# graz-dev/llms-on-kubernetes

Hardware: AMD Instinct MI355X
Metric: output tok/s through gateway (p50 TTFT reported) (higher is better)
Workload: dtype bf16

## Files before the change

csrc/include/hipserve/kernels.h:

```cpp
#pragma once
#include <hip/hip_runtime.h>
#include <stddef.h>

namespace hipserve {

void launch_embed_rmsnorm(void* out, void* residual, const void* table, const long* ids, const long* src,
                          const long* tok, const void* w, bool weight_f32, int rows, int hidden, float eps,
                          hipStream_t s, float scale = 1.f, void* out8 = nullptr, float* xs8 = nullptr);
void launch_rmsnorm(void* out, void* residual, const void* x, const void* w,
                    bool weight_f32, int rows, int hidden, long x_stride,
                    long out_stride, float eps, hipStream_t s, void* out8 = nullptr, float* xs8 = nullptr);
void launch_qk_rmsnorm(void* qkv, long stride, const float* qw, const float* kw, int T, int nq, int nkv, int D,
                       float eps, hipStream_t s);

void launch_silu_and_mul(void* out, const void* in, long rows, int inter,
                         long in_stride, long out_stride, hipStream_t s);
void launch_gelu_and_mul(void* out, const void* in, long rows, int inter,
                         long in_stride, long out_stride, hipStream_t s);

void launch_rope_cache(void* qkv, long qkv_stride, const long* positions,
                       const long* slots, const float* cos_sin, void* k_cache,
                       void* v_cache, int T, int nq, int nkv, int D,
                       int block_size, int mode, hipStream_t s, bool kv_f8 = false);

size_t paged_decode_smem_bytes(int D);
void launch_paged_decode_qkv(void* out, long out_stride, const float* ws, int S, int N, const long* positions,
                             const long* slots, const float* cos_sin, int mode, void* k_cache, void* v_cache,
                             const int* block_tables, int bt_stride, const int* context_lens, float* tmp_out,
                             float* tmp_ml, int B, int nq, int nkv, int D, int block_size, int part_size,
                             int max_parts, float scale, int window, hipStream_t s, void* out16 = nullptr,
                             const float* qw = nullptr, const float* kw = nullptr, float eps = 1e-6f);
void launch_paged_decode(void* out, long out_stride, const void* q, long q_stride,
                         const void* k_cache, const void* v_cache,
                         const int* block_tables, int bt_stride,
                         const int* context_lens, float* tmp_out, float* tmp_ml,
                         int B, int nq, int nkv, int D, int block_size,
                         int part_size, int max_parts, float scale, int window,
                         hipStream_t s, void* out16 = nullptr, bool kv_f8 = false);

void launch_prefill_attention(void* out, long out_stride, const void* q,
                              long q_stride, const void* k_cache,
                              const void* v_cache, const int* block_tables,
                              int bt_stride, const int* cu_q, const int* ctx_lens,
                              const int* tiles, int ntiles, int nq, int nkv, int D,
                              int block_size, float scale, int window, hipStream_t s, bool kv_f8 = false);

size_t sample_workspace_floats(int rows, int V);
void launch_sample(long* out_tok, float* out_lp, const void* logits, bool is_bf16,
                   long stride, int rows, int V, const float* temperature,
                   const int* top_k, const float* top_p, const long* seeds,
                   const long* steps, float* ws, hipStream_t s, bool two_rounds = true,
                   const float* min_p = nullptr);

void launch_penalty_apply(void* logits, bool is_bf16, long stride, int rows, int V, const int* slot,
                          const float* pres, const float* freq, const float* rep, const int* counts,
                          const unsigned int* seen, hipStream_t s);
void launch_logit_bias_apply(void* logits, bool is_bf16, long stride, int rows, int V, const int* slot,
                             const int* ids, const float* vals, const int* n, int nslots, int width,
                             hipStream_t s);
void launch_penalty_update(const long* tok, const int* slot, int n, int* counts, unsigned int* seen, int V,
                           hipStream_t s);
void launch_penalty_init(int* counts, unsigned int* seen, int V, const int* slots, const int* off,
                         const int* n_prompt, const int* toks, int ninit, hipStream_t s);
void launch_top_logprobs(const void* logits, bool is_bf16, long stride, int rows, int V, const int* nreq,
                         int* out_ids, float* out_lp, int K, hipStream_t s);

void launch_gguf_gemm(void* out, float* ws, const void* x, long x_stride, long out_stride,
                      const void* q, const void* d, const void* m, int qtype, long row_bytes,
                      int M, int N, int K, int splits, hipStream_t s);
void launch_gguf_dequant(void* out, const void* q, const void* d, const void* m, int qtype,
                         long row_bytes, int N, int K, hipStream_t s);
struct GgufPart {
  const void* q;
  const float* rs;
  int qtype;
  int rows;
  int col;
};
void launch_gguf_gemm_parts(void* out, long out_stride, float* ws, const void* x, long x_stride,
                            const GgufPart* parts, int nparts, int M, int Ntot, int K, int S, hipStream_t s,
                            const void* x16 = nullptr);
void launch_gguf_dequant_tiled(void* out, const void* q, const float* rs, int qtype, int N, int K, hipStream_t s,
                               int pack = 0, int nrows = 0, bool kmajor = false);
void launch_fp8_untile(void* out, const void* q, int N, int K, hipStream_t s);
bool launch_gguf_prefill(int epi, void* out, long ldo, const void* x16, const float* rsc, const GgufPart* parts,
                         int nparts, int M, int K, hipStream_t s);
void launch_x_f16_pairs(void* x16, float* rsc, const void* x, long ldx, int M, int K, hipStream_t s);
bool launch_qmoe_gemm(void* out, long out_stride, float* ws, const void* x, long x_stride, const void* q,
                      const float* rs, int qtype, long w_estride, long rs_estride, const int* slots,
                      const int* tile_expert, int tiles_cap, int tile, int gather_k, int N, int K, int S,
                      hipStream_t s, bool kmajor = false, int glu = 0);

}

namespace hipserve {
bool launch_skinny_gemm(void* out, const void* x, long x_stride, const void* w, long out_stride, int M,
                        int N, int K, int rt, int kw, hipStream_t s);

void* car_create(int rank, int world, size_t max_bytes, int nb_large);
void car_get_handle(void* state, void* handle_out);
void car_open(void* state, int peer, const void* handle);
bool car_error(void* state);
void car_destroy(void* state);
size_t car_max_bytes(void* state);
void launch_car(void* state, const void* inp, void* out, size_t bytes, bool two_shot, int blocks, hipStream_t s);
void launch_car_all_gather(void* state, const void* inp, void* out, size_t shard_bytes, size_t row_bytes,
                           hipStream_t s);
bool car_norm_fits(void* state, int M, int N, bool exch_f32);
void launch_car_add_rmsnorm(void* state, void* out, void* residual, const void* x, bool x_f32, int S,
                            const void* w, bool weight_f32, int M, int N, float eps, bool exch_f32, hipStream_t s);

void launch_fill_uniform(void* out, long ld, int rows, int cols, long row0, long col0, long gcols,
                         unsigned int key, float scale, hipStream_t s);

constexpr int DG_GLU = 1, DG_PARTIAL = 2;
bool launch_decode_gemm(void* out, long out_stride, float* ws, const void* x, long x_stride, const void* w, int M,
                        int N, int K, int rt, int S, bool packed, int flags, hipStream_t s);


constexpr int PG_EPI_STORE = 0, PG_EPI_ADD = 1, PG_EPI_GLU = 2, PG_EPI_GEGLU = 3;
constexpr int PW_EPI_STORE = 0, PW_EPI_ADD = 1, PW_EPI_GLU = 2, PW_EPI_GEGLU = 3;
struct PwGroup {
  const int* tile_expert;
  const int* num_tiles;
  long estride;
  const int* gather_slots = nullptr;
  int gather_k = 1;
  int x_rows = 0;
};
bool launch_prefill_gemm_packed(int epi, void* C, long ldc, const void* X, long ldx, const void* Wp, int M, int N,
                                int K, const void* bias, int wm, int grid_req, hipStream_t s,
                                const PwGroup* group = nullptr, int rw = 4);
constexpr int kPgF8Parts = 4;
struct PgF8Part {
  const unsigned char* q;
  const float* rs;
  int rows;
  int tile0;
};
struct PgF8 {
  PgF8Part p[kPgF8Parts];
  int n;
  const float* xs;
};
bool launch_prefill_gemm_f8(int epi, void* C, long ldc, const void* A, long lda, const PgF8& W, int M, int N, int K,
                            hipStream_t s);
bool launch_fp8_decode_gemm(float* ws, const void* xq, const PgF8& W, int M, int N, int K, int S, hipStream_t s);
bool launch_glu_quant(bool gelu, void* out, void* q8, float* xs, const void* in, long rows, int inter,
                      long in_stride, hipStream_t s);
void launch_act_quant_fp8(void* q, float* xs, const void* x, long x_stride, int M, int K, hipStream_t s);

void launch_splitk_add_rmsnorm(void* out, void* residual, const float* ws, int S, const void* w, bool weight_f32,
                               int M, int N, float eps, hipStream_t s, void* out16 = nullptr, void* out8 = nullptr,
                               float* xs8 = nullptr);
void launch_splitk_post_add_rmsnorm(void* out, void* residual, const float* ws, int S, const void* w_post,
                                    const void* w_next, bool weight_f32, int M, int N, float eps, hipStream_t s,
                                    void* out16 = nullptr, void* out8 = nullptr, float* xs8 = nullptr);
void launch_splitk_reduce(void* out, long out_stride, const float* ws, int M, int N, int S, hipStream_t s);
void launch_splitk_glu(void* act, long act_stride, const float* ws, int S, int M, int I, bool gelu, hipStream_t s,
                       void* act16 = nullptr);
void launch_splitk_rope_cache(void* qkv, long qkv_stride, const float* ws, int S, const long* positions,
                              const long* slots, const float* cos_sin, void* k_cache, void* v_cache, int T, int nq,
                              int nkv, int D, int block_size, int mode, hipStream_t s, const void* bias = nullptr,
                              const float* qw = nullptr, const float* kw = nullptr, float eps = 1e-6f,
                              bool kv_f8 = false);
void launch_pack_decode_weight(void* out, const void* w, int N, int K, bool glu, hipStream_t s, int batch = 1);
}

namespace hipserve {
void launch_moe_topk_softmax(const void* logits, bool logits_f32, float* w, int* ids, int T, int E, int k,
                             bool renorm, hipStream_t s, int splits = 0);
void launch_moe_align(const int* ids, int npairs, int E, int tile, int* slots, int slots_cap, int* tile_expert,
                      int tiles_cap, int* num_tiles, int* pair_slot, int* group_end, hipStream_t s,
                      int* hist = nullptr, int expert_lo = 0);
int moe_align_blocks(int npairs);
void launch_moe_gather(void* out, const void* x, long x_stride, const int* slots, int nslots, int k, int H,
// ... 37 lines not shown
```

csrc/kernels/rope_cache.hip:

```cpp
#include <cstdlib>

#include "hipserve/common.h"
#include "hipserve/kernels.h"

namespace hipserve {

template <int kMode>
HS_DEVICE void rotate8(float (&x)[8], float (&y)[8], const float* cs, int i0,
                       int half) {
#pragma unroll
  for (int j = 0; j < 8; ++j) {
    const float c = cs[i0 + j], s = cs[half + i0 + j];
    const float a = x[j], b = y[j];
    rope_rot(a, b, c, s, x[j], y[j]);
  }
}

template <int kMode, typename KV>
__global__ __launch_bounds__(256) void rope_cache_kernel(
    unsigned short* __restrict__ qkv, long qkv_stride,
    const long* __restrict__ positions, const long* __restrict__ slots,
    const float* __restrict__ cos_sin, KV* __restrict__ k_cache,
    KV* __restrict__ v_cache, int nq, int nkv, int D,
    int block_size) {
  const int t = blockIdx.x;
  const long pos = positions[t];
  const long slot = slots[t];
  const int half = D / 2;
  const float* cs = cos_sin + pos * D;
  unsigned short* row = qkv + t * qkv_stride;
  const long blk = slot >= 0 ? slot / block_size : 0;
  const int off = slot >= 0 ? (int)(slot % block_size) : 0;

  if constexpr (kMode == 0) {
    const int chunks = half / 8;
    const int items = (nq + nkv) * chunks;
    for (int it = threadIdx.x; it < items; it += blockDim.x) {
      const int h = it / chunks, c = it % chunks;
      unsigned short* base = row + h * D;
      u16x8 va = *reinterpret_cast<u16x8*>(base + c * 8);
      u16x8 vb = *reinterpret_cast<u16x8*>(base + half + c * 8);
      float x[8], y[8];
#pragma unroll
      for (int j = 0; j < 8; ++j) { x[j] = bf16_to_f32(va[j]); y[j] = bf16_to_f32(vb[j]); }
      rotate8<0>(x, y, cs, c * 8, half);
#pragma unroll
      for (int j = 0; j < 8; ++j) { va[j] = f32_to_bf16(x[j]); vb[j] = f32_to_bf16(y[j]); }
      if (h < nq) {
        *reinterpret_cast<u16x8*>(base + c * 8) = va;
        *reinterpret_cast<u16x8*>(base + half + c * 8) = vb;
      } else if (slot >= 0) {
        const int kh = h - nq;
        KV* kc = k_cache + ((blk * nkv + kh) * block_size + off) * (long)D;
        kv_store8(kc + c * 8, va);
        kv_store8(kc + half + c * 8, vb);
      }
    }
  } else {
    const int chunks = D / 8;
    const int items = (nq + nkv) * chunks;
    for (int it = threadIdx.x; it < items; it += blockDim.x) {
      const int h = it / chunks, c = it % chunks;
      unsigned short* base = row + h * D;
      u16x8 v = *reinterpret_cast<u16x8*>(base + c * 8);
#pragma unroll
      for (int p = 0; p < 4; ++p) {
        const int i = c * 4 + p;
        const float co = cs[i], si = cs[half + i];
        const float a = bf16_to_f32(v[2 * p]), b = bf16_to_f32(v[2 * p + 1]);
        float ra, rb;
        rope_rot(a, b, co, si, ra, rb);
        v[2 * p] = f32_to_bf16(ra);
        v[2 * p + 1] = f32_to_bf16(rb);
      }
      if (h < nq) {
        *reinterpret_cast<u16x8*>(base + c * 8) = v;
      } else if (slot >= 0) {
        const int kh = h - nq;
        KV* kc = k_cache + ((blk * nkv + kh) * block_size + off) * (long)D;
        kv_store8(kc + c * 8, v);
      }
    }
  }
  if (slot >= 0) {
    const unsigned short* vrow = row + (nq + nkv) * D;
    const int chunks = D / 8;
    for (int it = threadIdx.x; it < nkv * chunks; it += blockDim.x) {
      const int kh = it / chunks, c = it % chunks;
      const u16x8 v = *reinterpret_cast<const u16x8*>(vrow + kh * D + c * 8);
      KV* vc = v_cache + (blk * nkv + kh) * (long)D * block_size + off;
#pragma unroll
      for (int j = 0; j < 8; ++j) kv_store1(vc + (c * 8 + j) * block_size, v[j]);
    }
  }
}

constexpr int kRopeTile = 16;

template <int kMode, typename KV>
__global__ __launch_bounds__(256) void rope_cache_tile_kernel(
    unsigned short* __restrict__ qkv, long qkv_stride, const long* __restrict__ positions,
    const long* __restrict__ slots, const float* __restrict__ cos_sin, KV* __restrict__ k_cache,
    KV* __restrict__ v_cache, int T, int nq, int nkv, int D, int block_size, int vfast) {
  extern __shared__ __attribute__((aligned(16))) unsigned short vs[];
  const int t0 = blockIdx.x * kRopeTile;
  const int nt = min(kRopeTile, T - t0);
  const int half = D / 2;
  const int chunks = kMode == 0 ? half / 8 : D / 8;
  const int nh = nq + nkv;
  const int per_tok = chunks * 2;
  for (int it = threadIdx.x; it < nt * per_tok; it += blockDim.x) {
    const int tt = it / per_tok, c = (it % per_tok) >> 1, hpar = it & 1;
    const int t = t0 + tt;
    const long pos = positions[t];
    const long slot = slots[t];
    const float* cs = cos_sin + pos * D;
    unsigned short* row = qkv + t * qkv_stride;
    const long blk = slot >= 0 ? slot / block_size : 0;
    const int off = slot >= 0 ? (int)(slot % block_size) : 0;
    if constexpr (kMode == 0) {
      float co[8], si[8];
#pragma unroll
      for (int j = 0; j < 8; ++j) { co[j] = cs[c * 8 + j]; si[j] = cs[half + c * 8 + j]; }
      for (int h0 = hpar; h0 < nh; h0 += 8) {
        u16x8 va[4], vb[4];
#pragma unroll
        for (int q = 0; q < 4; ++q) {
          const int h = min(h0 + 2 * q, nh - 1);
          va[q] = *reinterpret_cast<const u16x8*>(row + h * D + c * 8);
          vb[q] = *reinterpret_cast<const u16x8*>(row + h * D + half + c * 8);
        }
#pragma unroll
        for (int q = 0; q < 4; ++q) {
          const int h = h0 + 2 * q;
          if (h >= nh || (h >= nq && slot < 0)) continue;
#pragma unroll
          for (int j = 0; j < 8; ++j) {
            float ra, rb;
            rope_rot(bf16_to_f32(va[q][j]), bf16_to_f32(vb[q][j]), co[j], si[j], ra, rb);
            va[q][j] = f32_to_bf16(ra);
            vb[q][j] = f32_to_bf16(rb);
          }
          if (h < nq) {
            *reinterpret_cast<u16x8*>(row + h * D + c * 8) = va[q];
            *reinterpret_cast<u16x8*>(row + h * D + half + c * 8) = vb[q];
          } else {
            KV* dst = k_cache + ((blk * nkv + (h - nq)) * block_size + off) * (long)D;
            kv_store8(dst + c * 8, va[q]);
            kv_store8(dst + half + c * 8, vb[q]);
          }
        }
      }
    } else {
      float co[4], si[4];
#pragma unroll
      for (int p = 0; p < 4; ++p) { co[p] = cs[c * 4 + p]; si[p] = cs[half + c * 4 + p]; }
      for (int h0 = hpar; h0 < nh; h0 += 8) {
        u16x8 v[4];
#pragma unroll
        for (int q = 0; q < 4; ++q)
          v[q] = *reinterpret_cast<const u16x8*>(row + min(h0 + 2 * q, nh - 1) * D + c * 8);
#pragma unroll
        for (int q = 0; q < 4; ++q) {
          const int h = h0 + 2 * q;
          if (h >= nh || (h >= nq && slot < 0)) continue;
#pragma unroll
          for (int p = 0; p < 4; ++p) {
            float ra, rb;
            rope_rot(bf16_to_f32(v[q][2 * p]), bf16_to_f32(v[q][2 * p + 1]), co[p], si[p], ra, rb);
            v[q][2 * p] = f32_to_bf16(ra);
            v[q][2 * p + 1] = f32_to_bf16(rb);
          }
          if (h < nq) *reinterpret_cast<u16x8*>(row + h * D + c * 8) = v[q];
          else kv_store8(k_cache + ((blk * nkv + (h - nq)) * block_size + off) * (long)D + c * 8, v[q]);
        }
      }
    }
  }
  const int VW = nkv * D, VR = VW + 8;
  const int vchunks = VW / 8;
  for (int it = threadIdx.x; it < nt * vchunks; it += blockDim.x) {
    const int tt = it / vchunks, c = it % vchunks;
    *reinterpret_cast<u16x8*>(vs + tt * VR + c * 8) =
        *reinterpret_cast<const u16x8*>(qkv + (t0 + tt) * qkv_stride + (nq + nkv) * D + c * 8);
  }
  __syncthreads();
  const long s0 = slots[t0];
  const int off0 = s0 >= 0 ? (int)(s0 % block_size) : 1;
  bool contig = vfast && nt == kRopeTile && (block_size & 7) == 0 && (off0 & 7) == 0 && off0 + kRopeTile <= block_size;
  for (int i = 1; contig && i < kRopeTile; ++i) contig = slots[t0 + i] == s0 + i;
  if (contig) {
    const long blk = s0 / block_size;
    for (int it = threadIdx.x; it < 2 * VW; it += blockDim.x) {
      const int r = it >> 1, hl = it & 1;
      const int kh = r / D, d = r % D;
      u16x8 v;
#pragma unroll
      for (int j = 0; j < 8; ++j) v[j] = vs[(hl * 8 + j) * VR + r];
      kv_store8(v_cache + (blk * nkv + kh) * (long)D * block_size + (long)d * block_size + off0 + hl * 8, v);
    }
    return;
  }
  const int tt = threadIdx.x & (kRopeTile - 1);
  const long slot = tt < nt ? slots[t0 + tt] : -1;
  if (slot < 0) return;
  const long blk = slot / block_size;
  const int off = (int)(slot % block_size);
  for (int r = threadIdx.x / kRopeTile; r < VW; r += blockDim.x / kRopeTile) {
    const int kh = r / D, d = r % D;
    kv_store1(v_cache + (blk * nkv + kh) * (long)D * block_size + (long)d * block_size + off, vs[tt * VR + r]);
  }
}

static bool rope_tile_enabled() {
  static const bool on = [] {
    const char* e = getenv("HIPSERVE_ROPE_TILE");
    return !(e && atoi(e) == 0);
  }();
  return on;
}

static int rope_vfast() {
  static const int on = [] {
    const char* e = getenv("HIPSERVE_ROPE_VFAST");
    return !(e && atoi(e) == 0) ? 1 : 0;
  }();
  return on;
}

template <typename KV>
static void rope_cache_t(unsigned short* q, long qkv_stride, const long* positions, const long* slots,
                         const float* cos_sin, KV* kc, KV* vc, int T, int nq, int nkv, int D, int block_size,
                         int mode, hipStream_t s) {
  if (T >= 2048 && nkv * D <= 2048 && rope_tile_enabled()) {
    const dim3 tg((T + kRopeTile - 1) / kRopeTile);
    const size_t smem = (size_t)kRopeTile * (nkv * D + 8) * sizeof(unsigned short);
    if (mode == 0)
      rope_cache_tile_kernel<0, KV><<<tg, 256, smem, s>>>(q, qkv_stride, positions, slots, cos_sin, kc, vc, T, nq,
                                                          nkv, D, block_size, rope_vfast());
    else
      rope_cache_tile_kernel<1, KV><<<tg, 256, smem, s>>>(q, qkv_stride, positions, slots, cos_sin, kc, vc, T, nq,
                                                          nkv, D, block_size, rope_vfast());
    return;
  }
  if (mode == 0)
    rope_cache_kernel<0, KV><<<T, 256, 0, s>>>(q, qkv_stride, positions, slots, cos_sin, kc, vc, nq, nkv, D,
                                               block_size);
  else
    rope_cache_kernel<1, KV><<<T, 256, 0, s>>>(q, qkv_stride, positions, slots, cos_sin, kc, vc, nq, nkv, D,
                                               block_size);
}

void launch_rope_cache(void* qkv, long qkv_stride, const long* positions,
                       const long* slots, const float* cos_sin, void* k_cache,
                       void* v_cache, int T, int nq, int nkv, int D,
                       int block_size, int mode, hipStream_t s, bool kv_f8) {
  if (T <= 0) return;
  auto* q = static_cast<unsigned short*>(qkv);
  if (kv_f8)
    rope_cache_t(q, qkv_stride, positions, slots, cos_sin, static_cast<unsigned char*>(k_cache),
                 static_cast<unsigned char*>(v_cache), T, nq, nkv, D, block_size, mode, s);
  else
    rope_cache_t(q, qkv_stride, positions, slots, cos_sin, static_cast<unsigned short*>(k_cache),
                 static_cast<unsigned short*>(v_cache), T, nq, nkv, D, block_size, mode, s);
}

}
```

csrc/torch_bindings.cpp:

```cpp
#include <torch/library.h>
#include <ATen/ATen.h>
#include <ATen/hip/impl/HIPGuardImplMasqueradingAsCUDA.h>
#include <ATen/hip/impl/HIPStreamMasqueradingAsCUDA.h>

#include <initializer_list>
#include <sstream>
#include <type_traits>

#include "hipserve/kernels.h"
#include "hipserve/quant_formats.h"

namespace {

hipStream_t cur_stream() {
  return c10::hip::getCurrentHIPStreamMasqueradingAsCUDA().stream();
}


enum : unsigned { BF16 = 1, F32 = 2, F16 = 4, U8 = 8, I8 = 16, I16 = 32, I32 = 64, I64 = 128, F8 = 256, OTHER = 512 };
constexpr unsigned BYTES = U8 | I8 | F8, ANYTYPE = ~0u;
struct DtypeName { unsigned bit; at::ScalarType type; const char* name; };
const DtypeName kDtypes[] = {{BF16, at::kBFloat16, "bf16"}, {F32, at::kFloat, "fp32"},  {F16, at::kHalf, "f16"},
                             {U8, at::kByte, "uint8"},      {I8, at::kChar, "int8"},    {I16, at::kShort, "int16"},
                             {I32, at::kInt, "int32"},      {I64, at::kLong, "int64"},  {F8, at::kFloat8_e4m3fn, "float8_e4m3fn"}};
// ... 221 lines not shown
    const int n = rs[i].numel();
    W.p[i] = hipserve::PgF8Part{a.as<uint8_t>(q[i], "q[i] (tiled FP8 [N/16, K/256, 4096] with rs [N])", CONTIG,
                                              exactly((int64_t)n * K)),
                                a.as<float>(rs[i], "rs[i]", CONTIG), n, tile0 ? rows / 256 : 0};
    rows += n;
  }
  return rows;
}

using hipserve::gq::QuantFormat;

std::string quant_formats() {
  std::ostringstream o;
  for (int id : hipserve::gq::kQuantFormatIds) {
    const QuantFormat f = hipserve::gq::quant_format(id);
    o << f.name << ' ' << f.id << ' ' << f.chunk_bytes << ' ' << f.sub_shift << ' ' << f.gguf << ' ' << f.row_scaled
      << ' ' << f.prefill << ' ' << f.moe << '\n';
  }
  return o.str();
}
QuantFormat tiled_format(int64_t qtype, const char* op, bool moe = false) {
  const QuantFormat f = hipserve::gq::quant_format(qtype == (int)qtype ? (int)qtype : -1);
  TORCH_CHECK(f.id >= 0 && (f.moe || !moe), op, ": kernel qtype ", qtype, moe ? " has no expert body" : " is unknown",
              "; name id chunk sub_shift gguf row_scaled prefill moe:\n", quant_formats());
  return f;
}

long tiled_parts(const Args& a, const std::vector<at::Tensor>& qs, const std::vector<at::Tensor>* rss,
                 const std::vector<int64_t>& qtypes, const std::vector<int64_t>& rows, const std::vector<int64_t>& cols,
                 int64_t K, hipserve::GgufPart* P) {
  const size_t np = qs.size();
  TORCH_CHECK(np >= 1 && np <= 4 && qtypes.size() == np && (!rss || rss->size() == np) && rows.size() == np &&
              cols.size() == np, a.op, ": 1-4 parts");
  long span = 0;
  for (size_t i = 0; i < np; ++i) {
    const QuantFormat f = tiled_format(qtypes[i], a.op);
    TORCH_CHECK(cols[i] >= 0 && cols[i] % 4 == 0 && rows[i] % 16 == 0 && rows[i] > 0, a.op,
                ": parts are 16-row multiples at 4-aligned columns");
    const void* q = a.ptr(qs[i], "qs[i] (a tiled [N/16, K/256, chunk] tensor of its format)", U8, CONTIG,
                          exactly(rows[i] / 16 * (K / 256) * f.chunk_bytes));
    const float* rs = rss && f.row_scaled ? a.as<float>((*rss)[i], "rss[i] (FP8 / INT8C: an fp32 scale per row)",
                                                         CONTIG, exactly(rows[i]))
                                          : nullptr;
    P[i] = hipserve::GgufPart{q, rs, (int)qtypes[i], (int)rows[i], (int)cols[i]};
    span = std::max(span, (long)(cols[i] + rows[i]));
  }
  return span;
}

struct GemmOut { void* out = nullptr; long stride = 0; float* ws = nullptr; };
GemmOut partials_or_out(const Args& a, const at::Tensor& out, const at::Tensor& ws, int64_t S, int64_t rows, int64_t N,
                        int64_t out_cols) {
  GemmOut o;
  o.ws = a.as_if<float>(ws, "ws", CONTIG, ws.numel() > 0 ? S * rows * N : 0);
  if (o.ws) return o;
  TORCH_CHECK(S == 1, a.op, ": split-K needs a partial workspace");
  o.out = a.ptr(out, "out", BF16, ROWS4, {rows, at_least(out_cols)});
  o.stride = out.stride(0);
  return o;
}

struct DecodeX { const void* p; int M, K; long stride; };
DecodeX decode_gemm_x(const Args& a, const at::Tensor& x, int64_t splits) {
  const void* p = a.ptr(x, "x", BF16, ROWS8, {ANY, ANY});
  const int M = x.size(0), K = x.size(1);
  TORCH_CHECK(M >= 1 && M <= 64, a.op, ": 1 <= M <= 64");
  TORCH_CHECK(splits >= 1 && K % (256 * splits) == 0, a.op, ": K must be a multiple of 256*splits");
  return {p, M, K, (long)x.stride(0)};
}

struct MoeTiles { int *slots, *tile_expert; long nslots; int tiles_cap; };
MoeTiles moe_tiles(const Args& a, const at::Tensor& slots, const at::Tensor& tile_expert, int64_t tile) {
  TORCH_CHECK(tile > 0, a.op, ": tile > 0");
  int* sp = a.as<int>(slots, "slots", CONTIG);
  const long nslots = slots.numel();
  return {sp, a.as<int>(tile_expert, "tile_expert", CONTIG, (nslots + tile - 1) / tile), nslots, (int)tile_expert.numel()};
}

struct Combine { const float* w; const int* pair_slot; };
Combine combine_args(const Args& a, const at::Tensor& w, const at::Tensor& pair_slot, int64_t pairs) {
  return {a.as<float>(w, "w", CONTIG, pairs), a.as<int>(pair_slot, "pair_slot", CONTIG, pairs)};
}

struct PenState { int* counts; unsigned int* seen; int V; };
PenState pen_state(const Args& a, const at::Tensor& counts, const at::Tensor& seen) {
  int* c = a.as<int>(counts, "counts", CONTIG, {ANY, ANY});
  const int V = counts.size(1);
  return {c, reinterpret_cast<unsigned int*>(a.as<int>(seen, "seen", CONTIG, {counts.size(0), (V + 31) / 32})), V};
}


void rmsnorm_op(const char* name, at::Tensor& out, const at::Tensor& x, at::Tensor* residual, const at::Tensor& weight,
                double eps, const c10::optional<at::Tensor>& out8, const c10::optional<at::Tensor>& xs8) {
  Args a(name, x, "x");
  const void* xp = a.ptr(x, "x", BF16, ROWS, {ANY, ANY});
  const int rows = x.size(0), hidden = x.size(1);
  TORCH_CHECK(hidden % 8 == 0 && hidden <= 16384, name, ": hidden must be a multiple of 8, <= 16384");
  void* op = a.ptr(out, "out", BF16, ROWS, {at_least(rows), at_least(hidden)});
  void* rp = residual ? a.ptr(*residual, "residual", BF16, CONTIG, {rows, hidden}) : nullptr;
  const NormWeight w = norm_weight(a, weight, "weight", hidden);
  const E4m3Out o8 = e4m3_out_args(a, out8, xs8, out);
  hipserve::launch_rmsnorm(op, rp, xp, w.p, w.f32, rows, hidden, x.stride(0), out.stride(0), (float)eps,
                           cur_stream(), o8.q, o8.xs);
}
void rmsnorm(at::Tensor& out, const at::Tensor& x, const at::Tensor& weight, double eps,
             const c10::optional<at::Tensor>& out8, const c10::optional<at::Tensor>& xs8) {
  rmsnorm_op("rmsnorm", out, x, nullptr, weight, eps, out8, xs8);
}
void fused_add_rmsnorm(at::Tensor& out, const at::Tensor& x, at::Tensor& residual, const at::Tensor& weight, double eps,
                       const c10::optional<at::Tensor>& out8, const c10::optional<at::Tensor>& xs8) {
  rmsnorm_op("fused_add_rmsnorm", out, x, &residual, weight, eps, out8, xs8);
}

void embed_rmsnorm(at::Tensor& out, at::Tensor& residual, const at::Tensor& table, const at::Tensor& ids,
                   const c10::optional<at::Tensor>& src, const c10::optional<at::Tensor>& tok,
                   const at::Tensor& weight, double eps, double scale, const c10::optional<at::Tensor>& out8,
                   const c10::optional<at::Tensor>& xs8) {
  Args a("embed_rmsnorm", table, "table");
  const void* tp = a.ptr(table, "table", BF16, CONTIG, {ANY, ANY});
  const int64_t* idp = a.as<int64_t>(ids, "ids", CONTIG);
  const int hidden = table.size(1), rows = ids.numel();
  TORCH_CHECK(hidden % 8 == 0 && hidden <= 16384, "embed_rmsnorm: hidden must be a multiple of 8, <= 16384");
  void* op = a.ptr(out, "out", BF16, CONTIG, {rows, hidden});
  void* rp = a.ptr(residual, "residual", BF16, CONTIG, {rows, hidden});
  TORCH_CHECK(src.has_value() == tok.has_value(), "embed_rmsnorm: src and tok come together");
  const int64_t *sp = nullptr, *kp = nullptr;
  if (src.has_value()) {
    sp = a.as<int64_t>(*src, "src", CONTIG, exactly(rows));
    kp = a.as<int64_t>(*tok, "tok", CONTIG);
  }
  const NormWeight w = norm_weight(a, weight, "weight", hidden);
  const E4m3Out o8 = e4m3_out_args(a, out8, xs8, out);
  hipserve::launch_embed_rmsnorm(op, rp, tp, idp, sp, kp, w.p, w.f32, rows, hidden, (float)eps, cur_stream(),
                                 (float)scale, o8.q, o8.xs);
}

using GluLauncher = void (*)(void*, const void*, long, int, long, long, hipStream_t);
void glu_and_mul(const char* name, GluLauncher launch, at::Tensor& out, const at::Tensor& x) {
  Args a(name, x, "x");
  const void* xp = a.ptr(x, "x", BF16, ROWS, {ANY, ANY});
  TORCH_CHECK(x.size(1) % 16 == 0, name, ": x [rows, 2 I], I % 8 == 0");
  void* op = a.ptr(out, "out", BF16, ROWS, {x.size(0), x.size(1) / 2});
  launch(op, xp, x.size(0), out.size(1), x.stride(0), out.stride(0), cur_stream());
}
void silu_and_mul(at::Tensor& out, const at::Tensor& x) {
  glu_and_mul("silu_and_mul", &hipserve::launch_silu_and_mul, out, x);
}
void gelu_and_mul(at::Tensor& out, const at::Tensor& x) {
  glu_and_mul("gelu_and_mul", &hipserve::launch_gelu_and_mul, out, x);
}

void rope_cache(at::Tensor& qkv, const at::Tensor& positions, const at::Tensor& slots,
                const at::Tensor& cos_sin, at::Tensor& k_cache, at::Tensor& v_cache,
                int64_t nq, int64_t nkv, int64_t head_dim, int64_t mode) {
  Args a("rope_cache", qkv, "qkv");
  TORCH_CHECK(head_dim > 0 && head_dim % 16 == 0 && (mode == 0 || mode == 1), "rope_cache: head_dim % 16 == 0, mode 0 / 1");
  void* qp = a.ptr(qkv, "qkv", BF16, ROWS, {ANY, at_least((nq + 2 * nkv) * head_dim)});
  const int T = qkv.size(0);
  const RopeArgs r = rope_args(a, positions, slots, cos_sin, T, head_dim);
  const KvCache kv = kv_cache(a, k_cache, v_cache, nkv, head_dim);
  hipserve::launch_rope_cache(qp, qkv.stride(0), r.positions, r.slots, r.cos_sin, kv.k, kv.v, T, nq, nkv, head_dim,
                              kv.bs, mode, cur_stream(), kv.f8);
}

void paged_decode(at::Tensor& out, const at::Tensor& q, const at::Tensor& k_cache,
                  const at::Tensor& v_cache, const at::Tensor& block_tables,
                  const at::Tensor& context_lens, at::Tensor& tmp_out, at::Tensor& tmp_ml,
                  int64_t nq, int64_t nkv, int64_t part_size, double scale, int64_t window,
                  const c10::optional<at::Tensor>& out16) {
  Args a("paged_decode", q, "q");
  const KvCache kv = kv_cache(a, k_cache, v_cache, nkv);
  const int D = kv.D;
  TORCH_CHECK(D == 64 || D == 96 || D == 128 || D == 256, "paged_decode: head_dim 64/96/128/256");
  const void* qp = a.ptr(q, "q", BF16, ROWS, {ANY, at_least(nq * D)});
  const int B = q.size(0);
  void* op = a.ptr(out, "out", BF16, ROWS, {at_least(B), at_least(nq * D)});
  const DecodeAttn g = decode_attn_args(a, block_tables, context_lens, tmp_out, tmp_ml, B, nq, nkv, D, kv.bs,
                                        part_size, window);
  hipserve::launch_paged_decode(op, out.stride(0), qp, q.stride(0), kv.k, kv.v, g.block_tables, g.bt_stride,
                                g.context_lens, g.tmp_out, g.tmp_ml, B, nq, nkv, D, kv.bs, part_size, g.max_parts,
                                (float)scale, (int)window, cur_stream(), out16_arg(a, out16, out), kv.f8);
}

void paged_decode_qkv(at::Tensor& out, const at::Tensor& ws, int64_t splits, const at::Tensor& positions,
                      const at::Tensor& slots, const at::Tensor& cos_sin, at::Tensor& k_cache, at::Tensor& v_cache,
                      const at::Tensor& block_tables, const at::Tensor& context_lens, at::Tensor& tmp_out,
                      at::Tensor& tmp_ml, int64_t nq, int64_t nkv, int64_t part_size, double scale, int64_t window,
                      int64_t mode, const c10::optional<at::Tensor>& out16, const c10::optional<at::Tensor>& q_w,
                      const c10::optional<at::Tensor>& k_w, double eps) {
  Args a("paged_decode_qkv", ws, "ws");
  const KvCache kv = kv_cache(a, k_cache, v_cache, nkv);
  const int D = kv.D;
  TORCH_CHECK(!kv.f8, "paged_decode_qkv: bf16 KV cache only");
  TORCH_CHECK(D == 64 || D == 128, "paged_decode_qkv: head_dim 64/128");
  TORCH_CHECK(mode == 0 || mode == 1, "paged_decode_qkv: mode 0 / 1");
  const float *qwp, *kwp;
  if (qk_norm_weights(a, q_w, k_w, D, &qwp, &kwp))
    TORCH_CHECK(mode == 0, "paged_decode_qkv: q/k norm needs rotate-half RoPE (mode 0)");
  void* op = a.ptr(out, "out", BF16, ROWS, {ANY, at_least(nq * D)});
  const int B = out.size(0);
  const long N = (nq + 2 * nkv) * D;
  const float* wsp = splitk_ws(a, ws, splits, B, N);
  const RopeArgs r = rope_args(a, positions, slots, cos_sin, B, D);
  const DecodeAttn g = decode_attn_args(a, block_tables, context_lens, tmp_out, tmp_ml, B, nq, nkv, D, kv.bs,
                                        part_size, window);
  hipserve::launch_paged_decode_qkv(op, out.stride(0), wsp, splits, N, r.positions, r.slots, r.cos_sin, mode, kv.k,
                                    kv.v, g.block_tables, g.bt_stride, g.context_lens, g.tmp_out, g.tmp_ml, B, nq,
                                    nkv, D, kv.bs, part_size, g.max_parts, (float)scale, (int)window, cur_stream(),
                                    out16_arg(a, out16, out), qwp, kwp, (float)eps);
}

void prefill_attention(at::Tensor& out, const at::Tensor& q, const at::Tensor& k_cache,
                       const at::Tensor& v_cache, const at::Tensor& block_tables,
                       const at::Tensor& cu_q, const at::Tensor& ctx_lens,
                       const at::Tensor& tiles, int64_t nq, int64_t nkv, double scale, int64_t window) {
  Args a("prefill_attention", q, "q");
  const KvCache kv = kv_cache(a, k_cache, v_cache, nkv);
  const int D = kv.D;
  TORCH_CHECK(D == 64 || D == 96 || D == 128 || D == 256, "prefill_attention: head_dim 64/96/128/256");
  TORCH_CHECK(window >= 0, "prefill_attention: window >= 0");
  TORCH_CHECK(kv.bs % 16 == 0 && nq % nkv == 0, "prefill_attention: block_size % 16 == 0, nq % nkv == 0");
  const void* qp = a.ptr(q, "q", BF16, ROWS, {ANY, at_least(nq * D)});
  void* op = a.ptr(out, "out", BF16, ROWS, {ANY, at_least(nq * D)});
  const int* bt = a.as<int>(block_tables, "block_tables", ROWS, {ANY, ANY});
  const int* cu = a.as<int>(cu_q, "cu_q", ROWS);
  const int* cl = a.as<int>(ctx_lens, "ctx_lens", ROWS);
  const int* tp = a.as<int>(tiles, "tiles", CONTIG, {ANY, 2});
  hipserve::launch_prefill_attention(op, out.stride(0), qp, q.stride(0), kv.k, kv.v, bt, block_tables.stride(0), cu, cl,
                                     tp, tiles.size(0), nq, nkv, D, kv.bs, (float)scale, (int)window, cur_stream(),
                                     kv.f8);
}

void qk_rmsnorm(at::Tensor& qkv, const at::Tensor& q_w, const at::Tensor& k_w, int64_t nq, int64_t nkv,
                int64_t head_dim, double eps) {
  Args a("qk_rmsnorm", qkv, "qkv");
  TORCH_CHECK(head_dim > 0 && head_dim <= 256, "qk_rmsnorm: head_dim <= 256");
  void* qp = a.ptr(qkv, "qkv", BF16, ROWS, {ANY, at_least((nq + nkv) * head_dim)});
  const float* qw = a.as<float>(q_w, "q_w", CONTIG, exactly(head_dim));
  const float* kw = a.as<float>(k_w, "k_w", CONTIG, exactly(head_dim));
  hipserve::launch_qk_rmsnorm(qp, qkv.stride(0), qw, kw, qkv.size(0), nq, nkv, head_dim, (float)eps, cur_stream());
}

void sample(at::Tensor& out_tok, at::Tensor& out_lp, const at::Tensor& logits,
            const at::Tensor& temperature, const at::Tensor& top_k, const at::Tensor& top_p,
            const at::Tensor& seeds, const at::Tensor& steps, bool two_rounds,
            const c10::optional<at::Tensor>& min_p) {
  Args a("sample", logits, "logits");
  const Logits L = logits_rows(a, logits);
  const int rows = L.rows;
  int64_t* tok = a.as<int64_t>(out_tok, "out_tok", CONTIG, rows);
  float* lp = a.as_if<float>(out_lp, "out_lp", CONTIG, out_lp.numel() > 0 ? rows : 0);
  const float* temp = a.as<float>(temperature, "temperature", CONTIG, rows);
  const int* tk = a.as<int>(top_k, "top_k", CONTIG, rows);
  const float* tpp = a.as<float>(top_p, "top_p", CONTIG, rows);
  const int64_t* sd = a.as<int64_t>(seeds, "seeds", CONTIG, rows);
  const int64_t* st = a.as<int64_t>(steps, "steps", CONTIG, rows);
  const float* minp = maybe(min_p).defined() ? a.as<float>(*min_p, "min_p", CONTIG, rows) : nullptr;
  const size_t wsn = hipserve::sample_workspace_floats(rows, L.V);
  at::Tensor ws;
  if (wsn) ws = at::empty({(long)wsn}, logits.options().dtype(at::kFloat));
  hipserve::launch_sample(tok, lp, L.p, L.bf16, L.stride, rows, L.V, temp, tk, tpp, sd, st,
                          wsn ? a.as<float>(ws, "workspace", CONTIG) : nullptr, cur_stream(), two_rounds, minp);
}

void gguf_gemm(at::Tensor& out, const at::Tensor& x, const at::Tensor& q, const at::Tensor& d,
               const at::Tensor& mn, int64_t qtype, int64_t row_bytes, int64_t N, int64_t K,
               at::Tensor& ws, int64_t splits) {
  Args a("gguf_gemm", x, "x");
  TORCH_CHECK(K > 0 && K % 256 == 0, "gguf_gemm: K must be a multiple of 256");
  TORCH_CHECK(qtype >= 0 && qtype <= 6, "gguf_gemm: qtype 0..6");
  const void* xp = a.ptr(x, "x", BF16, ROWS8, {ANY, at_least(K)});
  const int M = x.size(0);
  TORCH_CHECK(M <= 64, "gguf_gemm handles M <= 64 (use gguf_dequant + GEMM above)");
  void* op = a.ptr(out, "out", BF16, ROWS, {M, at_least(N)});
  const void* qp = a.ptr(q, "q", U8, CONTIG);
  const void* dp = a.ptr_if(d, "d (SoA scales)", I16 | F16, CONTIG, qtype <= 2 ? N * (K / 32) : 0);
  const void* mp = a.ptr_if(mn, "m (SoA mins)", I16 | F16, CONTIG, qtype == 1 ? N * (K / 32) : 0);
  float* wp = splits > 1 ? splitk_ws(a, ws, splits, M, N) : nullptr;
  hipserve::launch_gguf_gemm(op, wp, xp, x.stride(0), out.stride(0), qp, dp, mp, qtype, row_bytes, M, N, K, splits,
                             cur_stream());
}

int64_t gguf_gemm_parts(at::Tensor& out, at::Tensor& ws, const at::Tensor& x, const std::vector<at::Tensor>& qs,
                        const std::vector<at::Tensor>& rss, const std::vector<int64_t>& qtypes, const std::vector<int64_t>& rows,
                        const std::vector<int64_t>& cols, int64_t Ntot, int64_t K, int64_t splits,
                        const c10::optional<at::Tensor>& x16) {
  Args a("gguf_gemm_parts", x, "x");
  TORCH_CHECK(K > 0 && K % 256 == 0 && splits >= 1, "gguf_gemm_parts: K % 256 == 0, splits >= 1");
  const void* xp = a.ptr(x, "x", BF16, ROWS8, {ANY, at_least(K)});
  const int M = x.size(0);
  TORCH_CHECK(M >= 1, "gguf_gemm_parts: M >= 1 (M > 64 sweeps 64-row tiles)");
  const int nsb = K / 256;
  const int per = (nsb + splits - 1) / splits;
  const int S = (nsb + per - 1) / per;
  hipserve::GgufPart P[4];
  TORCH_CHECK(tiled_parts(a, qs, &rss, qtypes, rows, cols, K, P) <= Ntot, "gguf_gemm_parts: parts must lie inside Ntot");
  const GemmOut o = partials_or_out(a, out, ws, S, M, Ntot, Ntot);
  const void* x16p = f16_twin(a, x16, "x16", x, at_least(K));
  hipserve::launch_gguf_gemm_parts(o.out, o.stride, o.ws, xp, x.stride(0), P, (int)qs.size(), M, Ntot, K, splits,
                                   cur_stream(), x16p);
  return S;
}

void x_f16_pairs(at::Tensor& x16, at::Tensor& rsc, const at::Tensor& x) {
  Args a("x_f16_pairs", x, "x");
  const void* xp = a.ptr(x, "x", BF16, ROWS8, {ANY, ANY});
  const int M = x.size(0);
  void* x16p = a.ptr(x16, "x16", F16, CONTIG, {M, ANY});
  const int K = x16.size(1);
  TORCH_CHECK(K % 8 == 0 && x.size(1) >= K, "x_f16_pairs: x16 [M, K], K % 8, x rows of >= K");
  float* rp = a.as<float>(rsc, "rsc", CONTIG, M);
  if (M == 0) return;
  hipserve::launch_x_f16_pairs(x16p, rp, xp, x.stride(0), M, K, cur_stream());
}

// ... 516 lines not shown
  at::Tensor hist;
  if (nb > 1) hist = at::empty({(long)nb * 128}, ids.options().dtype(at::kInt));
  hipserve::launch_moe_align(ip, npairs, E, tile, t.slots, t.nslots, t.tile_expert,
                             t.tiles_cap, ntp, psp, ge, cur_stream(), nb > 1 ? a.as<int>(hist, "histogram", CONTIG) : nullptr,
                             (int)expert_lo);
}

void moe_gather(at::Tensor& out, const at::Tensor& x, const at::Tensor& slots, int64_t k) {
  Args a("moe_gather", x, "x");
  const int* sp = a.as<int>(slots, "slots", CONTIG);
  void* op = a.ptr(out, "out", BF16, CONTIG, {at_least(slots.numel()), ANY});
  const int H = out.size(1);
  const void* xp = a.ptr(x, "x", BF16, ROWS8, {ANY, H});
  TORCH_CHECK(H % 8 == 0, "moe_gather: H % 8 == 0");
  hipserve::launch_moe_gather(op, xp, x.stride(0), sp, slots.numel(), k, H, cur_stream());
}

void moe_gemm(at::Tensor& out, const at::Tensor& x, const at::Tensor& w, const at::Tensor& slots,
              const at::Tensor& tile_expert, int64_t tile, int64_t gather_k) {
  Args a("moe_gemm", x, "x");
  const void* wp = a.ptr(w, "w", BF16, CONTIG, {ANY, ANY, ANY});
  const int N = w.size(1), K = w.size(2);
  TORCH_CHECK(K % 256 == 0, "moe_gemm: K % 256 == 0");
  const MoeTiles t = moe_tiles(a, slots, tile_expert, tile);
  const void* xp = a.ptr(x, "x", BF16, ROWS8, {ANY, at_least(K)});
  void* op = a.ptr(out, "out", BF16, ROWS, {at_least(t.nslots), at_least(N)});
  TORCH_CHECK(gather_k > 0 || x.size(0) >= t.nslots, "moe_gemm: ungathered x needs one row per slot");
  hipserve::launch_moe_gemm(op, out.stride(0), xp, x.stride(0), wp, t.slots, t.tile_expert, t.nslots / tile, tile,
                            gather_k, N, K, cur_stream());
}

void moe_combine(at::Tensor& out, const at::Tensor& y, const at::Tensor& w, const at::Tensor& pair_slot,
                 int64_t k) {
  Args a("moe_combine", y, "y");
  void* op = a.ptr(out, "out", BF16, CONTIG, {ANY, ANY});
  const int T = out.size(0), H = out.size(1);
  TORCH_CHECK(H % 8 == 0, "moe_combine: H % 8 == 0");
  const void* yp = a.ptr(y, "y", BF16, CONTIG, {ANY, H});
  const Combine c = combine_args(a, w, pair_slot, T * k);
  hipserve::launch_moe_combine(op, yp, c.w, c.pair_slot, T, k, H, cur_stream());
}

void moe_decode_gemm(at::Tensor& out, const at::Tensor& x, const at::Tensor& w, const at::Tensor& slots,
                     const at::Tensor& tile_expert, int64_t tile, int64_t gather_k, int64_t N, int64_t splits,
                     bool packed, bool glu) {
  Args a("moe_decode_gemm", x, "x");
  TORCH_CHECK(tile == 16 || tile == 32 || tile == 64, "moe_decode_gemm: tile in {16, 32, 64}");
  const void* xp = a.ptr(x, "x", BF16, ROWS8, {ANY, ANY});
  const long K = x.size(1);
  TORCH_CHECK(K % 256 == 0 && splits >= 1 && K % (256 * splits) == 0, "moe_decode_gemm: K must be a multiple of 256 * splits");
  const MoeTiles t = moe_tiles(a, slots, tile_expert, tile);
  TORCH_CHECK(t.nslots % tile == 0, "moe_decode_gemm: slots in whole tiles");
  const void* wp = a.ptr(w, "w", BF16, CONTIG);
  TORCH_CHECK(w.dim() >= 2, "moe_decode_gemm: w [E, ...]");
  const long estride = packed ? (N + 127) / 128 * 128 * K : N * K;
  TORCH_CHECK(w.numel() == w.size(0) * estride, "moe_decode_gemm: weight size != E * (packed) N * K");
  TORCH_CHECK(gather_k > 0 || x.size(0) >= t.nslots, "moe_decode_gemm: ungathered x needs one row per slot");
  void* op;
  float* ws = nullptr;
  long out_stride = N;
  if (a.check(out, "out", F32 | BF16, ROWS) == F32) {
    TORCH_CHECK(!glu && N % 4 == 0, "moe_decode_gemm: fp32 partials [splits, slots, N] take no glu, N % 4 == 0");
    op = ws = a.as<float>(out, "out (fp32 partials [splits, slots, N])", CONTIG, splits * t.nslots * N);
    if (out.dim() == 2) out_stride = out.stride(0);
  } else {
    TORCH_CHECK(splits == 1, "moe_decode_gemm: bf16 out [slots, N] (glu: [slots, N/2]) needs splits == 1");
    TORCH_CHECK(!glu || N % 128 == 0, "moe_decode_gemm: glu needs N % 128 == 0");
    op = a.ptr(out, "out", BF16, ROWS4, {at_least(t.nslots), at_least(glu ? N / 2 : N)});
    out_stride = out.stride(0);
  }
  TORCH_CHECK(hipserve::launch_moe_decode_gemm(op, out_stride, ws, xp, x.stride(0), wp, estride, t.slots, t.tile_expert,
                                               t.nslots / tile, tile, gather_k, N, K, splits, packed, glu, cur_stream()),
              "moe_decode_gemm: unsupported K / splits (K / splits / 256 in {1,2,3,4,6,7,8,16}) or glu without packing");
}

void moe_combine_partial(at::Tensor& out, const at::Tensor& ws, const at::Tensor& w, const at::Tensor& pair_slot,
                         int64_t k) {
  Args a("moe_combine_partial", ws, "ws");
  void* op = a.ptr(out, "out", BF16, CONTIG, {ANY, ANY});
  const int T = out.size(0), H = out.size(1);
  TORCH_CHECK(H % 8 == 0, "moe_combine_partial: H % 8 == 0");
  const float* wsp = a.as<float>(ws, "ws", CONTIG, {ANY, ANY, H});
  const Combine c = combine_args(a, w, pair_slot, T * k);
  hipserve::launch_moe_combine_partial(op, wsp, ws.stride(0), ws.size(0), c.w, c.pair_slot, T, k, H, cur_stream());
}

void moe_combine_add_rmsnorm(at::Tensor& out, at::Tensor& residual, const at::Tensor& y, int64_t splits,
                             const at::Tensor& w, const at::Tensor& pair_slot, int64_t k, const at::Tensor& norm_w,
                             double eps) {
  Args a("moe_combine_add_rmsnorm", y, "y");
  void* op = a.ptr(out, "out", BF16, CONTIG, {ANY, ANY});
  const int T = out.size(0), H = out.size(1);
  TORCH_CHECK(H % 8 == 0 && H <= 16384, "moe_combine_add_rmsnorm: H must be a multiple of 8, <= 16384");
  void* rp = a.ptr(residual, "residual", BF16, CONTIG, {T, H});
  const Combine c = combine_args(a, w, pair_slot, T * k);
  const NormWeight nw = norm_weight(a, norm_w, "norm_w", H);
  const void* yp = splits > 0 ? a.ptr(y, "y (fp32 partials [S, slots, H])", F32, CONTIG, {at_least(splits), ANY, H})
                              : a.ptr(y, "y", BF16, CONTIG, {ANY, H});
  const long slab = splits > 0 ? y.stride(0) : 0;
  hipserve::launch_moe_combine_add_rmsnorm(op, rp, yp, slab, (int)splits, c.w, c.pair_slot, T, k, H, nw.p, nw.f32,
                                           (float)eps, cur_stream());
}

void layernorm(at::Tensor& out, const at::Tensor& x, const at::Tensor& w, const at::Tensor& b,
               const c10::optional<at::Tensor>& residual, double eps) {
  Args a("layernorm", x, "x");
  const void* xp = a.ptr(x, "x", BF16, CONTIG, {ANY, ANY});
  const int rows = x.size(0), C = x.size(1);
  TORCH_CHECK(C % 8 == 0 && C <= 8192, "layernorm: C must be a multiple of 8, <= 8192");
  void* op = a.ptr(out, "out", BF16, CONTIG, {rows, C});
  const void* wp = a.ptr(w, "w", BF16, CONTIG, exactly(C));
  const void* bp = a.ptr(b, "b", BF16, CONTIG, exactly(C));
  void* rp = maybe(residual).defined() ? a.ptr(*residual, "residual", BF16, CONTIG, {rows, C}) : nullptr;
  hipserve::launch_layernorm(op, rp, xp, wp, bp, rows, C, (float)eps, cur_stream());
}

void gelu_(at::Tensor& x, bool tanh_approx) {
  Args a("gelu_", x, "x");
  void* xp = a.ptr(x, "x", BF16, CONTIG);
  TORCH_CHECK(x.numel() % 8 == 0, "gelu_: numel must be a multiple of 8");
  hipserve::launch_gelu(xp, x.numel(), tanh_approx, cur_stream());
}

void vision_attention(at::Tensor& out, at::Tensor& qkv, const at::Tensor& cos_sin, const at::Tensor& cu,
                      const at::Tensor& tiles, int64_t nh, int64_t D, double scale) {
  Args a("vision_attention", qkv, "qkv");
  TORCH_CHECK(D == 16 || D == 64 || D == 72 || D == 80 || D == 96 || D == 128,
              "vision_attention: head_dim must be one of 16, 64, 72, 80, 96, 128");
  void* qp = a.ptr(qkv, "qkv", BF16, CONTIG, {ANY, 3 * nh * D});
  const int T = qkv.size(0);
  void* op = a.ptr(out, "out", BF16, CONTIG, {T, nh * D});
  const float* cs = a.as<float>(cos_sin, "cos_sin", CONTIG, {at_least(T), D});
  const int* cup = a.as<int>(cu, "cu", CONTIG);
  const int* tp = a.as<int>(tiles, "tiles", CONTIG, {ANY, 2});
  hipserve::launch_vision_attention(op, qp, cs, cup, tp, tiles.size(0), T, nh, D, (float)scale, cur_stream());
}

}

#define GPU_KEY_OPS(X) \
  X(moe_topk_softmax, "(Tensor(a!) w, Tensor(b!) ids, Tensor logits, int k, bool renorm=True, int splits=0) -> ()") \
  X(moe_combine_add_rmsnorm, "(Tensor(a!) out, Tensor(b!) residual, Tensor y, int splits, Tensor w, Tensor pair_slot, int k, Tensor norm_w, float eps) -> ()") \
  X(moe_align, "(Tensor ids, int E, int tile, Tensor(a!) slots, Tensor(b!) tile_expert, Tensor(c!) num_tiles, Tensor(d!) pair_slot, Tensor(e!)? group_end=None, int expert_lo=0) -> ()") \
  X(moe_gather, "(Tensor(a!) out, Tensor x, Tensor slots, int k) -> ()") \
  X(moe_gemm, "(Tensor(a!) out, Tensor x, Tensor w, Tensor slots, Tensor tile_expert, int tile, int gather_k) -> ()") \
  X(moe_combine, "(Tensor(a!) out, Tensor y, Tensor w, Tensor pair_slot, int k) -> ()") \
  X(moe_decode_gemm, "(Tensor(a!) out, Tensor x, Tensor w, Tensor slots, Tensor tile_expert, int tile, int gather_k, int N, int splits, bool packed, bool glu) -> ()") \
  X(moe_combine_partial, "(Tensor(a!) out, Tensor ws, Tensor w, Tensor pair_slot, int k) -> ()") \
  X(rmsnorm, "(Tensor(a!) out, Tensor x, Tensor weight, float eps, Tensor(b!)? out8=None, Tensor(c!)? xs8=None) -> ()") \
  X(embed_rmsnorm, "(Tensor(a!) out, Tensor(b!) residual, Tensor table, Tensor ids, Tensor? src, Tensor? tok, " \
                   "Tensor weight, float eps, float scale=1.0, Tensor(c!)? out8=None, Tensor(d!)? xs8=None) -> ()") \
  X(fused_add_rmsnorm, "(Tensor(a!) out, Tensor x, Tensor(b!) residual, Tensor weight, float eps, Tensor(c!)? out8=None, Tensor(d!)? xs8=None) -> ()") \
  X(silu_and_mul, "(Tensor(a!) out, Tensor x) -> ()") \
  X(rope_cache, "(Tensor(a!) qkv, Tensor positions, Tensor slots, Tensor cos_sin, Tensor(b!) k_cache, Tensor(c!) v_cache, int nq, int nkv, int head_dim, int mode) -> ()") \
  X(paged_decode, "(Tensor(a!) out, Tensor q, Tensor k_cache, Tensor v_cache, Tensor block_tables, Tensor context_lens, Tensor(b!) tmp_out, Tensor(c!) tmp_ml, int nq, int nkv, int part_size, float scale, int window=0, Tensor(d!)? out16=None) -> ()") \
  X(prefill_attention, "(Tensor(a!) out, Tensor q, Tensor k_cache, Tensor v_cache, Tensor block_tables, Tensor cu_q, Tensor ctx_lens, Tensor tiles, int nq, int nkv, float scale, int window=0) -> ()") \
  X(qk_rmsnorm, "(Tensor(a!) qkv, Tensor q_w, Tensor k_w, int nq, int nkv, int head_dim, float eps) -> ()") \
  X(gelu_and_mul, "(Tensor(a!) out, Tensor x) -> ()") \
  X(gguf_gemm, "(Tensor(a!) out, Tensor x, Tensor q, Tensor d, Tensor m, int qtype, int row_bytes, int N, int K, Tensor(b!) ws, int splits) -> ()") \
  X(gguf_dequant, "(Tensor(a!) out, Tensor q, Tensor d, Tensor m, int qtype, int row_bytes, int N, int K) -> ()") \
  X(fill_uniform, "(Tensor(a!) out, int row0, int col0, int gcols, int key, float scale) -> ()") \
  X(decode_gemm, "(Tensor(a!) out, Tensor x, Tensor w, Tensor(b!) ws, int rt, int splits) -> ()") \
  X(decode_gemm_packed, "(Tensor(a!) out, Tensor x, Tensor wp, Tensor(b!) ws, int N, int rt, int splits) -> ()") \
  X(pack_decode_weight, "(Tensor(a!) out, Tensor w, bool glu=False) -> ()") \
  X(decode_gemm_partial, "(Tensor(a!) ws, Tensor x, Tensor w, int N, int rt, int splits, bool packed) -> ()") \
  X(decode_gemm_glu, "(Tensor(a!) act, Tensor x, Tensor wp, Tensor(b!) ws, int N, int rt, int splits) -> ()") \
  X(prefill_gemm_packed, "(Tensor(a!) out, Tensor x, Tensor wp, int N, int epi, Tensor? bias=None, int wm=1, int grid=0, int rw=4) -> ()") \
  X(prefill_gemm_packed_grouped, "(Tensor(a!) out, Tensor x, Tensor wp, int N, int epi, Tensor tile_expert, Tensor num_tiles, int wm=1, int rw=4, Tensor? gather_slots=None, int gather_k=1) -> ()") \
  X(prefill_gemm_f8, "(Tensor(a!) out, Tensor xq, Tensor xs, Tensor[] q, Tensor[] rs, int epi) -> ()") \
  X(fp8_decode_gemm, "(Tensor(a!) ws, Tensor xq, Tensor xs, Tensor[] q, Tensor[] rs, int splits) -> ()") \
  X(glu_quant, "(Tensor(a!)? out, Tensor(b!) q8, Tensor(c!) xs, Tensor x, bool gelu) -> ()") \
  X(act_quant_fp8, "(Tensor(a!) xq, Tensor(b!) xs, Tensor x) -> ()") \
  X(splitk_add_rmsnorm, "(Tensor(a!) out, Tensor(b!) residual, Tensor ws, int splits, Tensor weight, float eps, Tensor(c!)? out16=None, Tensor(d!)? out8=None, Tensor(e!)? xs8=None) -> ()") \
  X(splitk_post_add_rmsnorm, "(Tensor(a!) out, Tensor(b!) residual, Tensor ws, int splits, Tensor w_post, Tensor w_next, float eps, Tensor(c!)? out16=None, Tensor(d!)? out8=None, Tensor(e!)? xs8=None) -> ()") \
  X(splitk_glu, "(Tensor(a!) act, Tensor ws, int splits, bool gelu, Tensor(b!)? act16=None) -> ()") \
  X(paged_decode_qkv, "(Tensor(a!) out, Tensor ws, int splits, Tensor positions, Tensor slots, Tensor cos_sin, Tensor(b!) k_cache, Tensor(c!) v_cache, Tensor block_tables, Tensor context_lens, Tensor(d!) tmp_out, Tensor(e!) tmp_ml, int nq, int nkv, int part_size, float scale, int window, int mode, Tensor(f!)? out16=None, Tensor? q_norm=None, Tensor? k_norm=None, float eps=1e-6) -> ()") \
  X(splitk_reduce, "(Tensor(a!) out, Tensor ws, int splits) -> ()") \
  X(splitk_rope_cache, "(Tensor(a!) qkv, Tensor ws, int splits, Tensor positions, Tensor slots, Tensor cos_sin, Tensor(b!) k_cache, Tensor(c!) v_cache, int nq, int nkv, int head_dim, int mode, Tensor? bias=None, Tensor? q_w=None, Tensor? k_w=None, float eps=1e-6) -> ()") \
  X(skinny_gemm, "(Tensor(a!) out, Tensor x, Tensor w, int rt, int kw) -> ()") \
  X(penalty_apply, "(Tensor(a!) logits, Tensor slot, Tensor pres, Tensor freq, Tensor rep, Tensor counts, Tensor seen) -> ()") \
  X(logit_bias_apply, "(Tensor(a!) logits, Tensor slot, Tensor ids, Tensor vals, Tensor n) -> ()") \
  X(penalty_update, "(Tensor tok, Tensor slot, Tensor(a!) counts, Tensor(b!) seen) -> ()") \
  X(penalty_init, "(Tensor(a!) counts, Tensor(b!) seen, Tensor slots, Tensor off, Tensor n_prompt, Tensor toks) -> ()") \
  X(top_logprobs, "(Tensor logits, Tensor nreq, Tensor(a!) out_ids, Tensor(b!) out_lp) -> ()") \
  X(layernorm, "(Tensor(a!) out, Tensor x, Tensor w, Tensor b, Tensor(b!)? residual, float eps) -> ()") \
  X(gelu_, "(Tensor(a!) x, bool tanh_approx) -> ()") \
  X(vision_attention, "(Tensor(a!) out, Tensor(b!) qkv, Tensor cos_sin, Tensor cu, Tensor tiles, int nh, int D, float scale) -> ()") \
  X(sample, "(Tensor(a!) out_tok, Tensor(b!) out_lp, Tensor logits, Tensor temperature, Tensor top_k, Tensor top_p, Tensor seeds, Tensor steps, bool two_rounds=True, Tensor? min_p=None) -> ()")

TORCH_LIBRARY(hipserve, m) {
#define DEF_OP(name, schema) m.def(#name schema);
  GPU_KEY_OPS(DEF_OP)
#undef DEF_OP
  m.def("gguf_gemm_parts(Tensor(a!) out, Tensor(b!) ws, Tensor x, Tensor[] qs, Tensor[] rss, int[] qtypes, int[] rows, int[] cols, int Ntot, int K, int splits, Tensor? x16=None) -> int", &gguf_gemm_parts);
  m.def("gguf_prefill(Tensor(a!) out, Tensor x16, Tensor rsc, Tensor[] qs, int[] qtypes, int[] rows, int[] cols, int K, int epi) -> bool", &gguf_prefill);
  m.def("x_f16_pairs(Tensor(a!) x16, Tensor(b!) rsc, Tensor x) -> ()", &x_f16_pairs);
  m.def("gguf_dequant_tiled(Tensor(a!) out, Tensor q, Tensor rs, int qtype, int N, int K, int pack=0, int nrows=0, bool kmajor=False) -> ()",
        &gguf_dequant_tiled);
  m.def("fp8_untile(Tensor(a!) out, Tensor q, int N, int K) -> ()", &fp8_untile);
  m.def("quant_formats() -> str", &quant_formats);
  m.def("qmoe_gemm(Tensor(a!) out, Tensor(b!) ws, Tensor x, Tensor q, Tensor rs, int qtype, int N, int K, Tensor slots, Tensor tile_expert, int tile, int gather_k, int splits, bool kmajor=False, int glu=0) -> int", &qmoe_gemm);
  m.def("stage_copy(Tensor(a!)[] dst, Tensor[] src, int device) -> ()", &stage_copy);
  m.def("car_create(int rank, int world, int max_bytes, int nb_large=512) -> int", &car_create);
  m.def("car_handle(int state) -> Tensor", &car_handle);
  m.def("car_open(int state, int peer, Tensor handle) -> ()", &car_open);
  m.def("car_all_reduce(int state, Tensor inp, Tensor(a!) out, bool two_shot) -> ()", &car_all_reduce);
  m.def("car_all_gather(int state, Tensor inp, Tensor(a!) out) -> ()", &car_all_gather);
  m.def("car_norm_fits(int state, int M, int N, bool exch_f32) -> bool", &car_norm_fits);
  m.def("car_add_rmsnorm(int state, Tensor(a!) out, Tensor(b!) residual, Tensor x, int splits, Tensor weight, float eps, bool exch_f32) -> ()", &car_add_rmsnorm);
  m.def("car_error(int state) -> bool", &car_error);
  m.def("car_destroy(int state) -> ()", &car_destroy);
}

TORCH_LIBRARY_IMPL(hipserve, CUDA, m) {
#define IMPL_OP(name, schema) m.impl(#name, &name);
  GPU_KEY_OPS(IMPL_OP)
#undef IMPL_OP
}
```

hipserve/engine/model_runner.py:

```python
from __future__ import annotations

import logging
import math
import os
import time
from dataclasses import dataclass, field

import numpy as np
import torch

from ..config import EngineConfig, ModelConfig
from ..models.llama import AttnMeta, LlamaModel
from ..ops import get_ops
from ..parallel.comm import TPGroup
from ..runtime import native
from .request import MAX_LOGIT_BIAS
from .scheduler import SchedulerOutput

log = logging.getLogger("hipserve.runner")
PREFILL_TILE = 128
TOP_LOGPROBS = 20
GPU_HEAD_DIMS = (64, 96, 128, 256)
GRAPH_BUCKETS = [1, 2, 4, 8, 16, 24, 32, 48, 64, 80, 96, 112, 128, 160, 192, 224, 256, 320, 384, 448, 512]


@dataclass
class StepInputs:
    ids: np.ndarray
    positions: np.ndarray
    slots: np.ndarray
    num_prefill_tokens: int
    num_decode: int
    bt_prefill: np.ndarray | None
    cu_q: np.ndarray | None
    ctx_prefill: np.ndarray | None
    tiles: np.ndarray | None
    bt_decode: np.ndarray | None
    ctx_decode: np.ndarray | None
    logits_rows: np.ndarray
    temperature: np.ndarray
    top_k: np.ndarray
    top_p: np.ndarray
    seeds: np.ndarray
    steps: np.ndarray
    pen_slot: np.ndarray | None = None
    pen_vals: np.ndarray | None = None
    nlogprobs: np.ndarray | None = None
    pen_init: tuple | None = None
    top_logprobs: int = 0
    src: np.ndarray | None = None
    extra: dict = field(default_factory=dict)
    min_p: np.ndarray | None = None
    bias_slot: np.ndarray | None = None
    bias_init: tuple | None = None


def pad_table(times: dict, tol: float = 1.03) -> dict:
    pad, best_t, best_m = {}, float("inf"), None
    for m in sorted(times, reverse=True):
        if times[m] <= best_t * tol:
            best_t, best_m = min(times[m], best_t), m
        pad[m] = best_m
    return {m: p for m, p in pad.items() if p > m}


_PACKED_TIMING: dict = {}


class ModelRunner:
    def __init__(self, ecfg: EngineConfig, mcfg: ModelConfig, tp: TPGroup, device=None):
        self.ecfg = ecfg
        self.mcfg = mcfg
        self.tp = tp
        self.device = torch.device(device or tp.device or ecfg.device)
        if self.device.type == "cuda":
            if self.device.index is None:
                self.device = torch.device("cuda", torch.cuda.current_device())
            torch.cuda.set_device(self.device)
        self.dtype = {"bfloat16": torch.bfloat16, "bf16": torch.bfloat16, "auto": torch.bfloat16,
                      "float32": torch.float32, "fp32": torch.float32}[ecfg.dtype]
        if self.device.type == "cuda" and self.dtype != torch.bfloat16:
            raise ValueError("the gfx950 kernels run bf16 activations; use --dtype bfloat16")
        if self.device.type == "cuda" and mcfg.head_dim not in GPU_HEAD_DIMS:
            raise ValueError(f"{mcfg.name}: head_dim {mcfg.head_dim} has no gfx950 attention kernel "
                             f"(supported: {', '.join(map(str, GPU_HEAD_DIMS))})")
        self.ops = get_ops(self.device)
        self.max_model_len = min(ecfg.max_model_len or mcfg.max_position_embeddings,
                                 mcfg.max_position_embeddings)
        self.block_size = ecfg.block_size
        self.model = LlamaModel(mcfg, tp, self.device, self.dtype, self.ops, max_pos=self.max_model_len,
                                enable_expert_parallel=ecfg.enable_expert_parallel)
        if mcfg.num_experts and tp.world_size > 1:
            m = self.model
            log.info("rank %d/%d MoE sharding: %s (experts %d-%d of %d, width %d of %d)", tp.rank, tp.world_size,
                     m.moe_shard[0], m.expert_lo, m.expert_lo + m.num_local_experts - 1, mcfg.num_experts,
                     m.inter, mcfg.expert_size)
        self.model.decode_partition = ecfg.decode_partition
        self.model.block_size_hint = ecfg.block_size
        if ecfg.kv_fp8:
            self.model.kv_dtype = torch.float8_e4m3fn
            self.model.fused_qkv_attention = False
        t0 = time.time()
        self._load_weights()
        self.load_time = time.time() - t0
        from ..utils.faults import FaultInjector

        FaultInjector.from_env().on_init(tp.rank, tp.world_size)
        self.init_times = {"weights_s": round(self.load_time, 2)}
        t1 = time.time()
        if tp.world_size > 1:
            if "tp_exact_reduce" in ecfg.extra:
                tp.exact_reduce = bool(ecfg.extra["tp_exact_reduce"])
            if self.device.type == "cuda":
                H = mcfg.hidden_size
                msg = max(ecfg.max_num_batched_tokens * H * 2,
                          ecfg.max_num_seqs * self.model.vpad * 2, 8 << 20)
                if tp.ensure_custom_ar(msg):
                    tp.calibrate_collectives(H, ecfg.max_num_batched_tokens)
        self.init_times["collectives_s"] = round(time.time() - t1, 2)
        self.max_bs = min(ecfg.max_num_seqs, max(GRAPH_BUCKETS))
        self.buckets = [b for b in GRAPH_BUCKETS if b <= max(self.max_bs, 1)]
        if self.buckets[-1] < self.max_bs:
            self.buckets.append(self.max_bs)
        tp.rccl_floor_rows = max(tp.rccl_floor_rows, self.buckets[-1])
        t1 = time.time()
        self.gemm_report = []
        if self.device.type == "cuda" and ecfg.extra.get("gemm_autotune", True):
            from ..ops import gemm

            ms = [b for b in self.buckets if b <= 64]
            self.model.fused_decode = bool(ecfg.extra.get("fused_decode",
                                                          os.environ.get("HIPSERVE_FUSED_DECODE", "1") != "0"))
            fused = self.model.fused_gemm_shapes() if self.model.fused_decode else {}
            self.gemm_report = gemm.TUNER.tune(self.model.gemm_shapes(), self.device, ms, fused=fused)
            self.single_layout = None
            if ecfg.extra.get("packed_decode", True):
                why = self._single_layout_reason()
                if why:
                    n, freed = self.model.to_single_layout()
                    self.single_layout = {"reason": why, "weights": n, "row_major_gb_freed": round(freed / 2**30, 2)}
                else:
                    self.model.pack_decode_weights(gemm.TUNER.packed_shapes())
            shadow = ecfg.extra.get("quant_dense_shadow", os.environ.get("HIPSERVE_QUANT_SHADOW", "0") == "1")
            moes = self.model.quant_moes() if hasattr(self.model, "quant_moes") else []
            if moes and shadow:
                from ..ops import quant as Q

                total = torch.cuda.get_device_properties(self.device).total_memory
                self.quant_shadow_bytes = Q.make_moe_shadows(moes, self.device, (24 << 30) + total // 4)
            qws = self.model.quant_weights() if hasattr(self.model, "quant_weights") else []
            if qws:
                from ..ops import quant as Q

                self.gguf_split_report = Q.tune_splits(
                    qws, self.device, [m for m in Q.M_BUCKETS if m <= 64],
                    f8_ms=[m for m in Q.F8_M_BUCKETS if m <= max(64, max(self.buckets, default=1))])
                lm = getattr(self.model, "lm_head", None)
                self.qprefill_report = Q.tune_qprefill([w for w in qws if w is not lm], self.device,
                                                       min(ecfg.max_num_batched_tokens, 8192)) \
                    if Q.QPREFILL_MODE == "auto" else []
                total = torch.cuda.get_device_properties(self.device).total_memory
                self.quant_shadow_bytes = getattr(self, "quant_shadow_bytes", 0)
                if shadow:
                    gguf = ecfg.extra.get("gguf_dense_shadow", shadow)
                    self.quant_shadow_bytes += Q.make_dense_shadows(qws, self.device, (24 << 30) + total // 4,
                                                                    gguf=gguf)
                self.quant_shadow_bytes += Q.make_fp8_plain(qws, self.device, (24 << 30) + total // 4)
            if getattr(self.mcfg, "num_experts", 0) and hasattr(self.model, "tune_moe_prefill"):
                self.moe_prefill_report = self.model.tune_moe_prefill(min(ecfg.max_num_batched_tokens, 16384))
            torch.cuda.empty_cache()
        self.init_times["decode_gemm_tune_s"] = round(time.time() - t1, 2)
        t1 = time.time()
        self.prefill_pad = None
        if self.device.type == "cuda" and ecfg.extra.get("prefill_pad", True) and tp.rank == 0:
            self.prefill_pad = self._probe_prefill_pad()
        V = mcfg.vocab_size
        nslots = max(1, ecfg.max_num_seqs)
        self.pen_counts = torch.zeros(nslots, V, dtype=torch.int32, device=self.device)
        self.pen_seen = torch.zeros(nslots, (V + 31) // 32, dtype=torch.int32, device=self.device)
        self._free_pen = list(range(nslots - 1, -1, -1))
        self.bias_ids = torch.zeros(nslots, MAX_LOGIT_BIAS, dtype=torch.int32, device=self.device)
        self.bias_vals = torch.zeros(nslots, MAX_LOGIT_BIAS, dtype=torch.float32, device=self.device)
        self.bias_n = torch.zeros(nslots, dtype=torch.int32, device=self.device)
        self._free_bias = list(range(nslots - 1, -1, -1))
        self.init_times["pad_probe_s"] = round(time.time() - t1, 2)
        t1 = time.time()
        self.num_blocks = self._num_kv_blocks()
        self.kv = self.model.allocate_kv_cache(self.num_blocks, self.block_size)
        self.init_times["kv_alloc_s"] = round(time.time() - t1, 2)
        self.pad_block = self.num_blocks - 1
        self.width = -(-self.max_model_len // self.block_size)
        part = ecfg.decode_partition
        self.max_parts = -(-self.width * self.block_size // part)
        nq = self.model.nq
        self.tmp_out = torch.empty(self.max_bs, nq, self.max_parts, mcfg.head_dim,
                                   device=self.device, dtype=torch.float32)
        self.tmp_ml = torch.empty(self.max_bs, nq, self.max_parts, 2, device=self.device,
                                  dtype=torch.float32)
        self.stats = {"graph_steps": 0, "eager_steps": 0}
        self.graphs: dict[int, torch.cuda.CUDAGraph] = {}
        self.graph_pool = None
        self._static = None
        self.use_graphs = self.device.type == "cuda" and not ecfg.enforce_eager
        if self.use_graphs:
            self._capture_graphs()
        self.init_times["graph_capture_s"] = round(getattr(self, "graph_capture_time", 0.0), 2)
        self.init_times_ranks = tp.gather_obj(dict(self.init_times))

    def _load_weights(self):
        fmt = self.ecfg.load_format
        model = self.ecfg.model
        if fmt == "auto":
            from ..config import PRESETS

            key = model.lower().split("/")[-1]
            if key in PRESETS:
                fmt = "dummy"
            elif model.endswith(".gguf"):
                fmt = "gguf"
            else:
                fmt = "safetensors"
        quant = self.ecfg.extra.get("quantization")
        if fmt == "dummy" and quant:
            self.model.allocate_random_quant(quant, seed=self.ecfg.seed)
        elif fmt == "dummy":
            self.model.allocate_random(seed=self.ecfg.seed)
        elif fmt == "safetensors":
            from ..weights.safetensors_loader import load_hf_weights

            load_hf_weights(self.model, model)
        elif fmt == "gguf":
            from ..weights.gguf import load_gguf_weights

            load_gguf_weights(self.model, model)
        else:
            raise ValueError(f"unknown load_format {fmt}")
        self.load_format = fmt

    def _single_layout_reason(self) -> str | None:
        mode = os.environ.get("HIPSERVE_SINGLE_LAYOUT", self.ecfg.extra.get("single_layout", "auto"))
        m = self.model
        if str(mode) == "0" or not hasattr(m, "single_layout_ok") or not m.single_layout_ok():
            return None
        if str(mode) == "1":
            return "forced"
        from ..ops import gemm, pgemm

        lw = m.layers[0]
        ws = [w for w in (lw.wqkv, lw.wo, lw.wgu, lw.wd) if isinstance(w, torch.Tensor)]
        per_layer = sum(w.numel() * w.element_size() for w in ws if gemm.packable(*w.shape))
        need = per_layer * len(m.layers)
        free, total = torch.cuda.mem_get_info(self.device)
        margin = (free - need - (24 << 30) - total // 4) >> 20
        if self.tp.world_size > 1:
            margin = self.tp.min_int(int(margin))
        if margin < 0:
            return "memory"
        units = []
        for kind, w in (("plain", lw.wqkv), ("add", lw.wo), ("glu", lw.wgu), ("add", lw.wd)):
            if isinstance(w, torch.Tensor) and gemm.packable(*w.shape) and (kind != "glu" or w.shape[0] % 128 == 0):
                units.append((kind, w.shape[0], w.shape[1]))
        M = self.ecfg.max_num_batched_tokens
        if not units or self.tp.world_size > 1 or M < 2048:
            return None
        key = (tuple(units), M)
        r = _PACKED_TIMING.get(key)
        if r is None:
            from ..ops import tune_cache as TC

            r = TC.get(self.device, "packed_prefill", [units, M])
            if r is None:
                r = pgemm.tune_packed(units, M, self.device, self.ops)
                TC.put(self.device, "packed_prefill", [units, M], r)
# ... 137 lines not shown
            ctx_d = np.array([s.end for s in so.decode], dtype=np.int32)
        n = len(sample_seqs)
        n_pf = len(sample_seqs) - len(so.decode)
        temp = np.empty(n, np.float32)
        topk = np.empty(n, np.int32)
        topp = np.empty(n, np.float32)
        seeds = np.empty(n, np.int64)
        steps = np.empty(n, np.int64)
        pen_slot = pen_vals = nlp = pen_init = None
        minp = bias_slot = bias_init = None
        topn = 0
        init, binit = [], []
        for i, q in enumerate(sample_seqs):
            p = q.params
            temp[i] = p.temperature
            if p.min_p:
                if minp is None:
                    minp = np.zeros(n, np.float32)
                minp[i] = p.min_p
            if p.logit_bias:
                if bias_slot is None:
                    bias_slot = np.full(n, -1, np.int32)
                if q.bias_slot is None:
                    q.bias_slot = self._free_bias.pop()
                    binit.append(q)
                bias_slot[i] = q.bias_slot
            topk[i] = p.top_k if p.top_k > 0 else 0
            topp[i] = p.top_p
            seeds[i] = q.seed
            steps[i] = len(q.output_token_ids)
            if p.has_penalties:
                if pen_slot is None:
                    pen_slot = np.full(n, -1, np.int32)
                    pen_vals = np.zeros((3, n), np.float32)
                    pen_vals[2] = 1.0
                if q.pen_slot is None:
                    q.pen_slot = self._free_pen.pop()
                pen_slot[i] = q.pen_slot
                pen_vals[:, i] = (p.presence_penalty, p.frequency_penalty, p.repetition_penalty)
                if i < n_pf:
                    init.append(q)
            if p.logprobs:
                if nlp is None:
                    nlp = np.zeros(n, np.int32)
                nlp[i] = min(p.logprobs, TOP_LOGPROBS)
                topn = max(topn, int(nlp[i]))
        if init:
            ids_l = [q.prompt_token_ids + [t for t in q.output_token_ids if t >= 0] for q in init]
            off = np.zeros(len(init) + 1, np.int32)
            off[1:] = np.cumsum([len(x) for x in ids_l])
            pen_init = (np.array([q.pen_slot for q in init], np.int32), off,
                        np.array([q.num_prompt_tokens for q in init], np.int32),
                        np.fromiter((t for x in ids_l for t in x), np.int32, int(off[-1])))
        if binit:
            off = np.zeros(len(binit) + 1, np.int32)
            off[1:] = np.cumsum([len(q.params.logit_bias) for q in binit])
            bias_init = (np.array([q.bias_slot for q in binit], np.int32), off,
                         np.fromiter((t for q in binit for t, _ in q.params.logit_bias), np.int32, int(off[-1])),
                         np.fromiter((b for q in binit for _, b in q.params.logit_bias), np.float32, int(off[-1])))
        inp = StepInputs(ids, pos, slots, Tp, len(so.decode), bt_p, cu_q, ctx_p, tiles, bt_d, ctx_d,
                         np.array(rows, dtype=np.int64), temp, topk, topp, seeds, steps,
                         pen_slot, pen_vals, nlp, pen_init, topn,
                         min_p=minp, bias_slot=bias_slot, bias_init=bias_init)
        if any(s.seq.mm is not None for s in seqs):
            self._prepare_mm(seqs, inp)
        return inp

    def _prepare_mm(self, seqs, inp: StepInputs):
        pos = np.array(inp.positions, dtype=np.int64, copy=True)
        rope_rows, rope_pos, images = [], [], []
        t = 0
        for s in seqs:
            mm = s.seq.mm
            n = s.num_tokens
            if mm is not None:
                npr = s.seq.num_prompt_tokens
                a, b = s.start, min(s.end, npr)
                if a < b:
                    p3 = mm.pos3[:, a:b]
                    pos[t:t + b - a] = p3[0]
                    odd = np.nonzero((p3[0] != p3[1]) | (p3[0] != p3[2]))[0]
                    if odd.size:
                        rope_rows.append(odd + t)
                        rope_pos.append(p3[:, odd])
                    for (ia, ib), im in zip(mm.spans, mm.images):
                        lo, hi = max(ia, a), min(ib, b)
                        if lo < hi:
                            images.append((t + lo - a, lo - ia, hi - ia, im.pixels, tuple(im.grid), im.digest))
                if s.end > npr:
                    k0 = max(s.start, npr)
                    pos[t + k0 - s.start:t + n] = np.arange(k0, s.end) + mm.delta
            t += n
        inp.positions = pos
        if rope_rows or images:
            inp.extra["mm"] = {
                "rope_rows": np.concatenate(rope_rows) if rope_rows else np.zeros(0, np.int64),
                "rope_pos": np.concatenate(rope_pos, 1) if rope_pos else np.zeros((3, 0), np.int64),
                "images": images}

    def release(self, seq):
        if seq.pen_slot is not None:
            self._free_pen.append(seq.pen_slot)
            seq.pen_slot = None
        if seq.bias_slot is not None:
            self._free_bias.append(seq.bias_slot)
            seq.bias_slot = None

    def _fill_bias_slots(self, bias_init):
        slots, off, ids, vals = bias_init
        cnt = np.diff(off).astype(np.int32)
        for j, s in enumerate(slots):
            a, b = int(off[j]), int(off[j + 1])
            self.bias_ids[s, :b - a].copy_(torch.from_numpy(ids[a:b]))
            self.bias_vals[s, :b - a].copy_(torch.from_numpy(vals[a:b]))
            self.bias_n[s:s + 1].copy_(torch.from_numpy(cnt[j:j + 1]))

    def _t(self, a, dtype=None):
        if a is None:
            return None
        t = torch.from_numpy(np.ascontiguousarray(a))
        if self.device.type == "cuda":
            t = t.pin_memory().to(self.device, non_blocking=True)
        return t

    @property
    def max_graph_batch(self) -> int:
        return self.buckets[-1] if self.use_graphs else 0

    def graph_eligible(self, inp: StepInputs) -> bool:
        return (self.use_graphs and inp.num_prefill_tokens == 0 and inp.pen_init is None
                and inp.bias_init is None and 0 < inp.num_decode <= self.buckets[-1])

    @torch.inference_mode()
    def execute(self, inp: StepInputs):
        n = len(inp.logits_rows)
        if self.graph_eligible(inp):
            return self.wait(self.launch(inp))
        if inp.src is not None:
            raise RuntimeError("device-side input ids (lookahead) need the hipGraph decode path")
        self.stats["eager_steps"] += 1
        ids = self._t(inp.ids)
        meta = AttnMeta(
            num_prefill_tokens=inp.num_prefill_tokens, num_decode=inp.num_decode,
            positions=self._t(inp.positions), slot_mapping=self._t(inp.slots),
            bt_prefill=self._t(inp.bt_prefill), cu_q=self._t(inp.cu_q),
            ctx_prefill=self._t(inp.ctx_prefill), tiles=self._t(inp.tiles),
            bt_decode=self._t(inp.bt_decode), ctx_decode=self._t(inp.ctx_decode),
            tmp_out=self.tmp_out, tmp_ml=self.tmp_ml)
        if inp.num_decode > self.max_bs:
            meta.tmp_out = torch.empty(inp.num_decode, *self.tmp_out.shape[1:], device=self.device)
            meta.tmp_ml = torch.empty(inp.num_decode, *self.tmp_ml.shape[1:], device=self.device)
        if "mm" in inp.extra:
            self._attach_mm(inp.extra["mm"], meta, len(inp.ids))
        hidden = self.model.forward(ids, meta, self.kv)
        if n == 0:
            return np.zeros(0, np.int64), np.zeros(0, np.float32), None
        rows = self._t(inp.logits_rows)
        logits = self.model.compute_logits(hidden.index_select(0, rows))
        top = None
        if inp.top_logprobs:
            ti = torch.empty(n, TOP_LOGPROBS, dtype=torch.int32, device=self.device)
            tl = torch.empty(n, TOP_LOGPROBS, dtype=torch.float32, device=self.device)
            self.ops.top_logprobs(logits, self._t(inp.nlogprobs), ti, tl)
        if inp.bias_init is not None:
            self._fill_bias_slots(inp.bias_init)
        if inp.bias_slot is not None:
            self.ops.logit_bias_apply(logits, self._t(inp.bias_slot), self.bias_ids, self.bias_vals, self.bias_n)
        pslot = None
        if inp.pen_slot is not None:
            if inp.pen_init is not None:
                self.ops.penalty_init(self.pen_counts, self.pen_seen, *[self._t(a) for a in inp.pen_init])
            pslot = self._t(inp.pen_slot)
            pv = self._t(inp.pen_vals)
            self.ops.penalty_apply(logits, pslot, pv[0], pv[1], pv[2], self.pen_counts, self.pen_seen)
        tok = torch.empty(n, dtype=torch.long, device=self.device)
        lp = torch.empty(n, dtype=torch.float32, device=self.device)
        self.ops.sample(tok, lp, logits, self._t(inp.temperature), self._t(inp.top_k),
                        self._t(inp.top_p), self._t(inp.seeds), self._t(inp.steps), min_p=self._t(inp.min_p))
        if pslot is not None:
            self.ops.penalty_update(tok, pslot, self.pen_counts, self.pen_seen)
        if inp.top_logprobs:
            top = (ti.cpu().numpy(), tl.cpu().numpy())
        return tok.cpu().numpy(), lp.cpu().numpy(), top

    def _attach_mm(self, mm: dict, meta: AttnMeta, T: int):
        from ..models.vision import image_geometry
        from ..multimodal import mrope_cos_sin

        cfg = self.mcfg
        if len(mm["rope_rows"]):
            cs = self.model.cos_sin.index_select(0, meta.positions)
            rows = self._t(mm["rope_rows"])
            vals = mrope_cos_sin(mm["rope_pos"], cfg.head_dim, cfg.rope_theta, cfg.mrope_section)
            cs.index_copy_(0, rows, self._t(vals))
            meta.cos_sin = cs
            meta.positions = torch.arange(T, device=self.device)
        if not mm["images"]:
            return
        vis = self.model.visual
        uniq = {}
        for _, _, _, pixels, grid, digest in mm["images"]:
            uniq.setdefault(digest, (pixels, grid))
        geo = image_geometry([g for _, g in uniq.values()], vis.cfg)
        emb, ds_all = vis.forward(torch.from_numpy(np.concatenate([p for p, _ in uniq.values()])), geo)
        cache, off = {}, 0
        m2 = vis.cfg.spatial_merge_size ** 2
        for digest, (pixels, _) in uniq.items():
            n = pixels.shape[0] // m2
            cache[digest] = (emb[off:off + n], [d[off:off + n] for d in ds_all])
            off += n
        rows, embs, dss = [], [], []
        for row0, lo, hi, pixels, grid, digest in mm["images"]:
            e, ds = cache[digest]
            rows.append(torch.arange(row0, row0 + hi - lo))
            embs.append(e[lo:hi])
            dss.append([d[lo:hi] for d in ds])
        meta.mm_rows = torch.cat(rows).to(self.device)
        meta.mm_embeds = torch.cat(embs).to(self.model.dtype)
        meta.mm_deepstack = [torch.cat([d[j] for d in dss]).to(self.model.dtype) for j in range(len(dss[0]))]

    def _graph_forward(self, b: int, full: bool = True):
        st = self._static
        meta = AttnMeta(num_prefill_tokens=0, num_decode=b, positions=st["pos"][:b],
                        slot_mapping=st["slots"][:b], bt_decode=st["bt"][:b], ctx_decode=st["ctx"][:b],
                        tmp_out=self.tmp_out, tmp_ml=self.tmp_ml)
        meta.id_src = (st["src"][:b], st["tok"])
        hidden = self.model.forward(st["ids"][:b], meta, self.kv)
        logits = self.model.compute_logits(hidden)
        if full:
            self.ops.top_logprobs(logits, st["nlp"][:b], st["top_ids"][:b], st["top_lp"][:b])
            self.ops.logit_bias_apply(logits, st["bslot"][:b], self.bias_ids, self.bias_vals, self.bias_n)
            self.ops.penalty_apply(logits, st["pslot"][:b], st["pres"][:b], st["freq"][:b], st["rep"][:b],
                                   self.pen_counts, self.pen_seen)
        self.ops.sample(st["tok"][:b], st["lp"][:b], logits, st["temp"][:b], st["topk"][:b],
                        st["topp"][:b], st["seeds"][:b], st["steps"][:b], two_rounds=full, min_p=st["minp"][:b])
        if full:
            self.ops.penalty_update(st["tok"][:b], st["pslot"][:b], self.pen_counts, self.pen_seen)

    def _stage_in(self, b: int, sg):
        st, mb, W = self._static, self.buckets[-1], self.width
        torch.ops.hipserve.stage_copy([st["d64"], st["d32"][: b * W], st["d32"][mb * W:], st["df"]],
                                      [sg["h64"], sg["h32"][: b * W], sg["h32"][mb * W:], sg["hf"]],
                                      self.device.index or 0)

    def _stage_out(self, b: int, sg):
        st = self._static
        torch.ops.hipserve.stage_copy([sg["tok"][:b], sg["lp"][:b], sg["top_ids"][:b], sg["top_lp"][:b]],
                                      [st["tok"][:b], st["lp"][:b], st["top_ids"][:b], st["top_lp"][:b]],
                                      self.device.index or 0)

    @torch.inference_mode()
    def _capture_graphs(self):
        mb, W, dev = self.buckets[-1], self.width, self.device
        self._stage = []
        for _ in range(2):
            self._stage.append({
                "h64": torch.zeros(6 * mb, dtype=torch.long).pin_memory(),
                "h32": torch.zeros(mb * W + 5 * mb, dtype=torch.int32).pin_memory(),
                "hf": torch.zeros(6 * mb, dtype=torch.float32).pin_memory(),
                "tok": torch.zeros(mb, dtype=torch.long).pin_memory(),
                "lp": torch.zeros(mb, dtype=torch.float32).pin_memory(),
                "top_ids": torch.zeros(mb, TOP_LOGPROBS, dtype=torch.int32).pin_memory(),
                "top_lp": torch.zeros(mb, TOP_LOGPROBS, dtype=torch.float32).pin_memory(),
                "done": None,
                "bias_set": False, "minp_set": False,
            })
            self._stage[-1]["h32"][mb * W + 4 * mb:].fill_(-1)
        self._launches = 0
        self._stage_kernel = os.environ.get("HIPSERVE_STAGE_COPY", "kernel") != "blit"
        d64 = torch.zeros(6 * mb, dtype=torch.long, device=dev)
        d32 = torch.zeros(mb * W + 5 * mb, dtype=torch.int32, device=dev)
        df = torch.zeros(6 * mb, dtype=torch.float32, device=dev)
        st = {
            "d64": d64, "d32": d32, "df": df,
            "ids": d64[0:mb], "pos": d64[mb:2 * mb], "slots": d64[2 * mb:3 * mb],
            "seeds": d64[3 * mb:4 * mb], "steps": d64[4 * mb:5 * mb], "src": d64[5 * mb:6 * mb],
            "bt": d32[: mb * W].view(mb, W), "ctx": d32[mb * W: mb * W + mb],
            "topk": d32[mb * W + mb: mb * W + 2 * mb],
            "pslot": d32[mb * W + 2 * mb: mb * W + 3 * mb], "nlp": d32[mb * W + 3 * mb: mb * W + 4 * mb],
            "bslot": d32[mb * W + 4 * mb: mb * W + 5 * mb],
            "temp": df[0:mb], "topp": df[mb:2 * mb],
            "pres": df[2 * mb:3 * mb], "freq": df[3 * mb:4 * mb], "rep": df[4 * mb:5 * mb],
            "minp": df[5 * mb:6 * mb],
            "tok": torch.zeros(mb, dtype=torch.long, device=dev),
            "lp": torch.zeros(mb, dtype=torch.float32, device=dev),
            "top_ids": torch.zeros(mb, TOP_LOGPROBS, dtype=torch.int32, device=dev),
            "top_lp": torch.zeros(mb, TOP_LOGPROBS, dtype=torch.float32, device=dev),
        }
        self._static = st
        st["bt"].fill_(self.pad_block)
        st["ctx"].fill_(1)
        st["slots"].fill_(self.pad_block * self.block_size)
        st["topp"].fill_(1.0)
        st["src"].fill_(-1)
        st["pslot"].fill_(-1)
        st["bslot"].fill_(-1)
        st["rep"].fill_(1.0)
        t0 = time.time()
        self.tp.barrier()
        stream = torch.cuda.Stream(device=dev)
        stream.wait_stream(torch.cuda.current_stream(dev))
        with torch.cuda.stream(stream):
            self._graph_forward(self.buckets[-1])
            for b in reversed(self.buckets):
                for full in (True, False):
                    self._graph_forward(b, full)
        stream.synchronize()
        torch.cuda.synchronize(dev)
        self.tp.barrier()
        self.graph_pool = torch.cuda.graph_pool_handle()
        for b in reversed(self.buckets):
            for par in ((0, 1) if self._stage_kernel else (None,)):
                for full in (True, False):
                    g = torch.cuda.CUDAGraph()
                    with torch.cuda.graph(g, pool=self.graph_pool, stream=stream):
                        if par is not None:
                            self._stage_in(b, self._stage[par])
                        self._graph_forward(b, full)
                        if par is not None:
                            self._stage_out(b, self._stage[par])
                    self.graphs[(b, par, full)] = g
        torch.cuda.synchronize(dev)
        self.graph_capture_time = time.time() - t0

    @torch.inference_mode()
    def launch(self, inp: StepInputs):
        n = inp.num_decode
        b = next(x for x in self.buckets if x >= n)
        mb, W = self.buckets[-1], self.width
        self.stats["graph_steps"] += 1
        sg = self._stage[self._launches & 1]
        self._launches += 1
        if sg["done"] is not None:
            sg["done"].synchronize()
        h64, h32, hf = sg["h64"], sg["h32"], sg["hf"]
        pad_slot = self.pad_block * self.block_size
# ... 72 lines not shown
```

hipserve/models/llama.py:

```python
from __future__ import annotations

import math
import os
from dataclasses import dataclass

import torch
import torch.nn.functional as F

from ..config import ModelConfig
from ..ops import gemm, pgemm
from ..ops import quant as Q
from ..ops import reference as ref
from ..parallel.comm import TPGroup
from .moe import MOE_KERNEL_MAX_PAIRS, MOE_KERNEL_MAX_ROWS_PER_EXPERT, MoEMixin


@dataclass
class AttnMeta:
    num_prefill_tokens: int
    num_decode: int
    positions: torch.Tensor
    slot_mapping: torch.Tensor
    bt_prefill: torch.Tensor | None = None
    cu_q: torch.Tensor | None = None
    ctx_prefill: torch.Tensor | None = None
    tiles: torch.Tensor | None = None
    bt_decode: torch.Tensor | None = None
    ctx_decode: torch.Tensor | None = None
    tmp_out: torch.Tensor | None = None
    tmp_ml: torch.Tensor | None = None
    cos_sin: torch.Tensor | None = None
    mm_rows: torch.Tensor | None = None
    mm_embeds: torch.Tensor | None = None
    mm_deepstack: list | None = None
    id_src: tuple | None = None


@dataclass
class LayerWeights:
    ln1: torch.Tensor
    wqkv: torch.Tensor
    wo: torch.Tensor
    ln2: torch.Tensor
    wgu: torch.Tensor | None = None
    wd: torch.Tensor | None = None
    router: torch.Tensor | None = None
    w13: torch.Tensor | None = None
    w2: torch.Tensor | None = None
    moe_packed: tuple | None = None
    bqkv: torch.Tensor | None = None
    q_norm: torch.Tensor | None = None
    k_norm: torch.Tensor | None = None
    post_attn_norm: torch.Tensor | None = None
    post_ff_norm: torch.Tensor | None = None


def shard_sizes(cfg: ModelConfig, tp: int):
    assert cfg.num_heads % tp == 0, f"num_heads {cfg.num_heads} not divisible by TP {tp}"
    nq = cfg.num_heads // tp
    if cfg.num_kv_heads >= tp:
        assert cfg.num_kv_heads % tp == 0
        nkv = cfg.num_kv_heads // tp
    else:
        assert tp % cfg.num_kv_heads == 0
        nkv = 1
    I = cfg.expert_size if cfg.num_experts else cfg.intermediate_size
    assert I % tp == 0
    inter = I // tp
    vpad = (cfg.vocab_size + tp - 1) // tp
    return nq, nkv, inter, vpad


def moe_width_has_kernel(cfg: ModelConfig, tp: int) -> bool:
    return cfg.expert_size % tp == 0 and (cfg.expert_size // tp) % 256 == 0


def moe_sharding(cfg: ModelConfig, tp: int, enable_ep: bool = False, hip: bool = False, rank: int = 0):
    E = cfg.num_experts
    if tp == 1 or not E:
        return ("width", shard_sizes(cfg, tp)[2])
    shape = f"{cfg.name}: {E} experts of width {cfg.expert_size}"
    if enable_ep:
        if E % tp:
            raise ValueError(f"--enable-expert-parallel needs num_experts % TP == 0 ({shape}, TP={tp}: "
                             f"E={E}, tp={tp})")
        return ("expert", rank * (E // tp), E // tp)
    if not hip or moe_width_has_kernel(cfg, tp):
        return ("width", shard_sizes(cfg, tp)[2])
    if E % tp:
        raise ValueError(f"{shape} cannot run at TP={tp}: the width slice {cfg.expert_size}/{tp} has no gfx950 "
                         f"expert kernel (it needs a multiple of 256) and expert parallelism "
                         f"(--enable-expert-parallel) needs num_experts % TP == 0")
    return ("expert", rank * (E // tp), E // tp)


class LlamaModel(MoEMixin):
    native_fp8 = True
    fused_qkv_attention = os.environ.get("HIPSERVE_FUSED_QKV_ATTN", "1") == "1"

    def __init__(self, cfg: ModelConfig, tp: TPGroup, device, dtype=torch.bfloat16, ops=None,
                 max_pos: int | None = None, enable_expert_parallel: bool = False):
        self.cfg = cfg
        self.tp = tp
        self.device = torch.device(device)
        self.dtype = dtype
        self.kv_dtype = dtype
        self.ops = ops
        self.nq, self.nkv, self.inter, self.vpad = shard_sizes(cfg, tp.world_size)
        self.moe_shard = moe_sharding(cfg, tp.world_size, enable_expert_parallel,
                                      getattr(ops, "name", "") == "hip", tp.rank)
        self.expert_lo, self.num_local_experts = 0, cfg.num_experts
        if self.moe_shard[0] == "expert":
            _, self.expert_lo, self.num_local_experts = self.moe_shard
            self.inter = cfg.expert_size
        self.D = cfg.head_dim
        self.scale = cfg.attn_scale or 1.0 / math.sqrt(self.D)
        self.layers: list[LayerWeights] = []
        self.embed: torch.Tensor | None = None
        self.norm: torch.Tensor | None = None
        self.lm_head: torch.Tensor | None = None
        mp = max_pos or cfg.max_position_embeddings
        self.cos_sin = ref.rope_cos_sin(self.D, mp, cfg.rope_theta, cfg.rope_scaling).to(self.device)
        self.cos_sin_local = self.cos_sin
        if cfg.rope_local_theta and any(cfg.layer_windows):
            self.cos_sin_local = ref.rope_cos_sin(self.D, mp, cfg.rope_local_theta, None).to(self.device)
        self.fused_family = (cfg.hidden_act in ("silu", "gelu_tanh")
                             and (not cfg.qk_norm or (cfg.rope_mode == 0 and self.D in (64, 128, 256))))
        self.decode_partition = 512
        self.block_size_hint = 16
        self.quant_linear = None
        self.fused_decode = True
        self.visual = None
        if cfg.vision is not None:
            from .vision import VisionTower

            self.visual = VisionTower(cfg.vision, self.device, dtype, ops)

    def allocate_random(self, seed: int = 0, std: float = 0.02):
        cfg, dev, dt = self.cfg, self.device, self.dtype
        H, D = cfg.hidden_size, self.D
        rank, tp = self.tp.rank, self.tp.world_size
        scale = std * math.sqrt(3.0)
        names = {}

        def fill(view, key, row0, col0, gcols):
            k = (seed * 1000003 + names.setdefault(key, len(names) + 1) * 7919) & 0xFFFFFFFF
            self.ops.fill_uniform(view, row0, col0, gcols, k, scale)

        def new(*shape):
            return torch.empty(*shape, device=dev, dtype=dt)

        nd = torch.float32 if cfg.norm_offset else dt

        def ones(n, dtype=None):
            return torch.ones(n, device=dev, dtype=dtype or nd)

        self.embed = new(self.vpad, H)
        fill(self.embed, "embed", rank * self.vpad, 0, H)
        self.norm = ones(H)
        if cfg.tie_word_embeddings:
            self.lm_head = self.embed
        else:
            self.lm_head = new(self.vpad, H)
            fill(self.lm_head, "lm_head", rank * self.vpad, 0, H)
        nq, nkv, I = self.nq, self.nkv, self.inter
        kv_head0 = rank * nkv if cfg.num_kv_heads >= tp else rank // (tp // cfg.num_kv_heads)
        self.layers = []
        for li in range(cfg.num_layers):
            lw = LayerWeights(ln1=ones(H), wqkv=new((nq + 2 * nkv) * D, H), wo=new(H, nq * D), ln2=ones(H))
            fill(lw.wqkv[:nq * D], f"{li}.q", rank * nq * D, 0, H)
            fill(lw.wqkv[nq * D:(nq + nkv) * D], f"{li}.k", kv_head0 * D, 0, H)
            fill(lw.wqkv[(nq + nkv) * D:], f"{li}.v", kv_head0 * D, 0, H)
            fill(lw.wo, f"{li}.o", 0, rank * nq * D, cfg.num_heads * D)
            if cfg.qkv_bias:
                lw.bqkv = torch.zeros((nq + 2 * nkv) * D, device=dev, dtype=dt)
            if cfg.qk_norm:
                lw.q_norm, lw.k_norm = ones(D, torch.float32), ones(D, torch.float32)
            if cfg.sandwich_norm:
                lw.post_attn_norm, lw.post_ff_norm = ones(H), ones(H)
            if cfg.num_experts:
                E, Ig = cfg.num_experts, cfg.expert_size
                lw.router = new(E, H)
                fill(lw.router, f"{li}.router", 0, 0, H)
                lo, El = self.expert_lo, self.num_local_experts
                c0 = 0 if self.moe_shard[0] == "expert" else rank * I
                lw.w13 = new(El, 2 * I, H)
                lw.w2 = new(El, H, I)
                for j in range(El):
# ... 224 lines not shown
            lw.wqkv = conv(lw.wqkv)
            lw.wo = conv(lw.wo)
            if lw.wgu is not None:
                lw.wgu = conv(lw.wgu, glu=True)
                lw.wd = conv(lw.wd)
        if self.lm_head is not self.embed:
            self.lm_head = conv(self.lm_head)
        freed += self.pack_moe_weights(drop_plain=True)
        if self.device.type == "cuda":
            torch.cuda.empty_cache()
        return n, freed

    def fused_gemm_shapes(self) -> dict:
        if not self.layers or not self.fused_family:
            return {}
        lw = self.layers[0]
        out = {}
        dense = (torch.Tensor, gemm.PackedLinear)
        if isinstance(lw.wo, dense):
            out[tuple(lw.wo.shape)] = ("norm",)
        if isinstance(lw.wd, dense):
            out[tuple(lw.wd.shape)] = ("norm",)
        if isinstance(lw.wqkv, dense):
            kind = "attn" if self.fused_qkv_attn_ok() else "rope"
            out[tuple(lw.wqkv.shape)] = (kind, self.nq, self.nkv, self.D, self.cfg.rope_mode)
        if isinstance(lw.wgu, dense) and lw.wgu.shape[0] % 128 == 0 and self.cfg.hidden_act == "silu":
            out[tuple(lw.wgu.shape)] = ("glu",)
        return out

    def fused_qkv_attn_ok(self, layer: int | None = None) -> bool:
        lw0 = self.layers[0] if self.layers else None
        if (not self.fused_qkv_attention or self.D not in (64, 128) or lw0 is None or lw0.bqkv is not None
                or (lw0.q_norm is not None and self.cfg.rope_mode != 0)
                or torch.finfo(self.kv_dtype).bits != 16):
            return False
        layers = range(len(self.layers)) if layer is None else (layer,)
        return not any(self.cfg.window_of(i) for i in layers)

    def _fused_ok(self, meta: AttnMeta) -> bool:
        return (self.fused_decode and meta.num_prefill_tokens == 0
                and getattr(self.ops, "name", "") == "hip" and self.fused_family)

    def fused_embed_ok(self, meta: AttnMeta) -> bool:
        return (self._fused_ok(meta) and self.tp.world_size == 1 and self.embed.dtype == torch.bfloat16
                and hasattr(torch.ops.hipserve, "embed_rmsnorm"))

    @staticmethod
    def resolve_ids(ids: torch.Tensor, meta: AttnMeta) -> torch.Tensor:
        if meta.id_src is None:
            return ids
        src, tok = meta.id_src
        return torch.where(src >= 0, tok.index_select(0, src.clamp(min=0)), ids)

    def add_rmsnorm(self, out, residual, x, splits, w, out16=None, out8=None, out8p=None):
        eps = self.cfg.rms_norm_eps
        if self.tp.world_size > 1:
            assert out16 is None and out8 is None and out8p is None, "out16 / out8 need TP = 1"
            return self.tp.add_rmsnorm(out, residual, x, splits, w, eps, ops=self.ops)
        if x.dtype == torch.float32 and residual.dtype != torch.float32:
            q8, s8 = out8 if out8 is not None else (None, None)
            torch.ops.hipserve.splitk_add_rmsnorm(out, residual, x, splits, w, eps, out16, q8, s8)
        else:
            assert out16 is None and out8 is None, "out16 / out8 need the split-K partial path"
            self.ops.fused_add_rmsnorm(out, x, residual, w, eps, out8=out8p)
        return out

    def post_add_rmsnorm(self, out, residual, pt, x, w, w_post, w_next, out16=None, out8=None):
        eps = self.cfg.rms_norm_eps
        tp1 = self.tp.world_size == 1
        if tp1 and pt is not None and w_post.dtype == w_next.dtype and residual.dtype == torch.bfloat16:
            q8, s8 = out8 if out8 is not None else (None, None)
            torch.ops.hipserve.splitk_post_add_rmsnorm(out, residual, pt[0], pt[1], w_post, w_next, eps, out16, q8, s8)
            return True
        if pt is not None and not tp1 and self.tp.exact_reduce:
            S, (M, N) = pt[1], residual.shape
            o = pt[0].reshape(-1)[:S * M * N].view(S, M, N).sum(0)
        elif pt is not None:
            o = torch.empty_like(residual)
            torch.ops.hipserve.splitk_reduce(o, pt[0], pt[1])
        else:
            o = self.linear_rowpar(x, w)
        if not tp1:
            o = self._tp_sum(o, residual)
        self.ops.rmsnorm(o, o, w_post, eps)
        self.ops.fused_add_rmsnorm(out, o, residual, w_next, eps)
        return False

    def linear_rowpar(self, x: torch.Tensor, w) -> torch.Tensor:
        if (self.tp.world_size > 1 and self.tp.exact_reduce and x.is_cuda and isinstance(w, torch.Tensor)):
            return torch.mm(x, w.t(), out_dtype=torch.float32)
        return self.linear(x, w)

    def _tp_sum(self, x: torch.Tensor, like: torch.Tensor) -> torch.Tensor:
        self.tp.all_reduce(x)
        return x if x.dtype == like.dtype else x.to(like.dtype)

    def embed_tokens(self, ids: torch.Tensor) -> torch.Tensor:
        if self.tp.world_size == 1:
            return F.embedding(ids, self.embed)
        start = self.tp.rank * self.vpad
        local = ids - start
        mask = (local >= 0) & (local < self.vpad)
        h = F.embedding(local.clamp(0, self.vpad - 1), self.embed)
        h = h * mask.unsqueeze(-1).to(h.dtype)
        return self.tp.all_reduce(h)

    def _embed(self, ids: torch.Tensor, meta: AttnMeta) -> torch.Tensor:
        h = self.embed_tokens(self.resolve_ids(ids, meta))
        if self.cfg.embed_scale != 1.0:
            h = h * float(torch.tensor(self.cfg.embed_scale, dtype=h.dtype))
        return h

    def _rowpar_norm(self, xn, residual, x, w, post_w, next_w, x8, h=None, add=None):
        ops, eps, T = self.ops, self.cfg.rms_norm_eps, xn.shape[0]
        if h is None and add is None and post_w is None and self.tp.world_size == 1:
            epi = (gemm.packed_prefill if isinstance(w, gemm.PackedLinear) and T > 64
                   else Q.qprefill if Q.qprefill_ok(w, T) else None)
            if epi is not None:
                epi(x, w, 1, out=residual)
                return ops.rmsnorm(xn, residual, next_w, eps, out8=x8)
        if h is None:
            h = self.linear_rowpar(x, w)
        if add is not None and self.tp.rank == 0:
            h = h.index_add(0, add[0], add[1].to(h.dtype))
        if post_w is not None:
            h = self._tp_sum(h, xn)
            ops.rmsnorm(h, h, post_w, eps)
            ops.fused_add_rmsnorm(xn, h, residual, next_w, eps, out8=x8)
        else:
            self.add_rmsnorm(xn, residual, h, 1, next_w, out8p=x8)

    def forward(self, ids: torch.Tensor, meta: AttnMeta, kv_caches) -> torch.Tensor:
        ops, cfg = self.ops, self.cfg
        T = ids.shape[0]
        D, nq, nkv = self.D, self.nq, self.nkv
        eps = cfg.rms_norm_eps
        Tp, Td = meta.num_prefill_tokens, meta.num_decode
        if self._fused_ok(meta):
            return self.forward_decode_fused(ids, meta, kv_caches)
        h = self._embed(ids, meta)
        ds = None
        if meta.mm_rows is not None:
            h.index_copy_(0, meta.mm_rows, meta.mm_embeds.to(h.dtype))
            ds = meta.mm_deepstack
        cos_sin = self.cos_sin if meta.cos_sin is None else meta.cos_sin
        residual = h.clone()
        xn = torch.empty_like(h)
        attn = torch.empty(T, nq * D, device=h.device, dtype=h.dtype)
        if Td:
            part, tmp_out, tmp_ml = self._decode_split(Td, meta)
        x8 = self._x8p(xn, self.layers[0].wqkv)
        ops.rmsnorm(xn, h, self.layers[0].ln1, eps, out8=x8)
        L = len(self.layers)
        for i, lw in enumerate(self.layers):
            if x8 is not None:
                qkv = pgemm.f8_gemm(xn, lw.wqkv, 0, x8=x8)
            else:
                qkv = self.linear(xn, lw.wqkv)
            if lw.bqkv is not None:
                qkv += lw.bqkv
            if lw.q_norm is not None:
                ops.qk_rmsnorm(qkv, lw.q_norm, lw.k_norm, nq, nkv, D, eps)
            kc, vc = kv_caches[i]
            win = cfg.window_of(i)
            ops.rope_cache(qkv, meta.positions, meta.slot_mapping, self.cos_sin_local if win else cos_sin,
                           kc, vc, nq, nkv, D, cfg.rope_mode)
            if Tp:
                ops.prefill_attention(attn[:Tp], qkv[:Tp], kc, vc, meta.bt_prefill, meta.cu_q,
                                      meta.ctx_prefill, meta.tiles, nq, nkv, self.scale, win)
            if Td:
                ops.paged_decode(attn[Tp:Tp + Td], qkv[Tp:Tp + Td], kc, vc, meta.bt_decode, meta.ctx_decode,
                                 tmp_out, tmp_ml, nq, nkv, part, self.scale, win)
            x8 = self._x8p(xn, lw.wgu, glu=True)
            self._rowpar_norm(xn, residual, attn, lw.wo, lw.post_attn_norm, lw.ln2, x8)
            nxt = self.layers[i + 1].ln1 if i + 1 < L else self.norm
            x8n = self._x8p(xn, self.layers[i + 1].wqkv) if i + 1 < L else None
            act = h = None
            if lw.router is not None:
                h = self.moe(xn, lw)
            else:
                gelu = cfg.hidden_act == "gelu_tanh"
                if pgemm.f8_use(lw.wgu, T, glu=True):
                    act8 = None
                    if pgemm.f8_use(lw.wd, T):
                        act8 = pgemm.f8_glu_q8(xn, lw.wgu, gelu, x8)
                    if act8 is not None:
                        h = pgemm.f8_gemm(None, lw.wd, 0, x8=act8)
                    else:
                        act = pgemm.f8_gemm(xn, lw.wgu, 3 if gelu else 2, x8=x8)
                elif isinstance(lw.wgu, gemm.PackedLinear) and lw.wgu.glu:
                    act = gemm.packed_glu(xn, lw.wgu, gelu)
                elif cfg.hidden_act in ("silu", "gelu_tanh") and Q.qprefill_ok(lw.wgu, T, glu=True):
                    act = Q.qprefill(xn, lw.wgu, 3 if gelu else 2)
                if act is None and h is None:
                    gu = self.linear(xn, lw.wgu)
                    act = torch.empty(T, self.inter, device=xn.device, dtype=xn.dtype)
                    self.act_and_mul(act, gu)
            add = (meta.mm_rows, ds[i]) if ds is not None and i < len(ds) else None
            self._rowpar_norm(xn, residual, act, lw.wd, lw.post_ff_norm, nxt, x8n, h, add)
            x8 = x8n
        return xn

    def act_and_mul(self, out: torch.Tensor, gu: torch.Tensor):
        if self.cfg.hidden_act == "gelu_tanh":
            return self.ops.gelu_and_mul(out, gu)
        return self.ops.silu_and_mul(out, gu)

    def forward_decode_fused(self, ids: torch.Tensor, meta: AttnMeta, kv_caches) -> torch.Tensor:
        ops, cfg, op = self.ops, self.cfg, torch.ops.hipserve
        T = ids.shape[0]
        D, nq, nkv = self.D, self.nq, self.nkv
        eps = cfg.rms_norm_eps
        xn16 = None
        xn8 = None
        if ids.dtype == torch.long and self.fused_embed_ok(meta):
            residual = torch.empty(T, cfg.hidden_size, device=ids.device, dtype=self.embed.dtype)
            xn = torch.empty_like(residual)
            xn8 = self._x8(xn, self.layers[0].wqkv)
            src, tok = meta.id_src if meta.id_src is not None else (None, None)
            scale = float(torch.tensor(cfg.embed_scale, dtype=self.embed.dtype))
            op.embed_rmsnorm(xn, residual, self.embed, ids, src, tok, self.layers[0].ln1, eps, scale,
                             *(xn8 if xn8 is not None else (None, None)))
            h = residual
        else:
            h = self._embed(ids, meta)
            residual = h.clone()
            xn = torch.empty_like(h)
            ops.rmsnorm(xn, h, self.layers[0].ln1, eps)
        attn = torch.empty(T, nq * D, device=h.device, dtype=h.dtype)
        part, tmp_out, tmp_ml = self._decode_split(T, meta)
        one_part = -(-meta.bt_decode.shape[1] * self.block_size_hint // part) == 1
        L = len(self.layers)
        for i, lw in enumerate(self.layers):
            kc, vc = kv_caches[i]
            win = cfg.window_of(i)
            fuse_qa = one_part and self.fused_qkv_attn_ok(i) and kc.element_size() == 2
            cs = self.cos_sin_local if win else self.cos_sin
            pt = self._partial(xn, lw.wqkv, xn16, xn8)
            attn16 = self._x16(attn, lw.wo)
            if pt is not None and fuse_qa:
                op.paged_decode_qkv(attn, pt[0], pt[1], meta.positions, meta.slot_mapping, self.cos_sin, kc, vc,
                                    meta.bt_decode, meta.ctx_decode, tmp_out, tmp_ml, nq, nkv, part, self.scale,
                                    0, cfg.rope_mode, attn16, lw.q_norm, lw.k_norm, eps)
            elif pt is not None:
                ws, S = pt
                qkv = torch.empty(T, lw.wqkv.shape[0], device=h.device, dtype=h.dtype)
                op.splitk_rope_cache(qkv, ws, S, meta.positions, meta.slot_mapping, cs, kc, vc,
                                     nq, nkv, D, cfg.rope_mode, lw.bqkv, lw.q_norm, lw.k_norm, eps)
            else:
                qkv = self.linear(xn, lw.wqkv)
                if lw.bqkv is not None:
                    qkv += lw.bqkv
                if lw.q_norm is not None:
                    ops.qk_rmsnorm(qkv, lw.q_norm, lw.k_norm, nq, nkv, D, eps)
                ops.rope_cache(qkv, meta.positions, meta.slot_mapping, cs, kc, vc, nq, nkv, D,
                               cfg.rope_mode)
            if pt is None or not fuse_qa:
                ops.paged_decode(attn, qkv, kc, vc, meta.bt_decode, meta.ctx_decode, tmp_out, tmp_ml,
                                 nq, nkv, part, self.scale, win, attn16)
            xn16, xn8 = self._decode_rowpar_norm(xn, residual, attn, lw.wo, attn16, lw.post_attn_norm, lw.ln2, lw.wgu)
            nxt = self.layers[i + 1].ln1 if i + 1 < L else self.norm
            if lw.router is not None:
                tail = ((xn, residual, nxt) if self.tp.world_size == 1 and self.ops.name == "hip"
                        and residual.dtype == torch.bfloat16 else None)
                y = self.moe(xn, lw, tail=tail)
                if y is not None:
                    self.add_rmsnorm(xn, residual, y, 1, nxt)
                continue
            gelu = cfg.hidden_act == "gelu_tanh"
            gc = None if gelu else gemm.glu_choice(T, lw.wgu)
            pt = (None if gc is not None or (isinstance(lw.wgu, torch.Tensor) and not gelu)
                  else self._partial(xn, lw.wgu, xn16, xn8))
            act16 = None
            if gc is not None:
                act = gemm.gemm_glu(xn, lw.wgu, gc)
            elif pt is not None:
                act = torch.empty(T, self.inter, device=xn.device, dtype=xn.dtype)
                act16 = self._x16(act, lw.wd)
                op.splitk_glu(act, pt[0], pt[1], gelu, act16)
            elif isinstance(lw.wgu, gemm.PackedLinear) and lw.wgu.glu:
                act = gemm.packed_glu(xn, lw.wgu, gelu)
            else:
                gu = self.linear(xn, lw.wgu)
                act = torch.empty(T, self.inter, device=xn.device, dtype=xn.dtype)
                self.act_and_mul(act, gu)
            consumer = self.layers[i + 1].wqkv if i + 1 < L else None
            xn16, xn8 = self._decode_rowpar_norm(xn, residual, act, lw.wd, act16, lw.post_ff_norm, nxt, consumer)
        return xn

    def _decode_rowpar_norm(self, xn, residual, x, w, x16, post_w, next_w, consumer):
        pt = self._partial(x, w, x16)
        xn16 = self._x16(xn, consumer) if pt is not None else None
        xn8 = self._x8(xn, consumer) if pt is not None else None
        if post_w is not None:
            if not self.post_add_rmsnorm(xn, residual, pt, x, w, post_w, next_w, xn16, xn8):
                xn16 = xn8 = None
        elif pt is not None:
            self.add_rmsnorm(xn, residual, pt[0], pt[1], next_w, xn16, xn8)
        else:
            self.add_rmsnorm(xn, residual, self.linear_rowpar(x, w), 1, next_w)
        return xn16, xn8

    def quant_weights(self) -> list:
        ws = [self.lm_head] + [getattr(lw, n) for lw in self.layers for n in ("wqkv", "wo", "wgu", "wd")]
        return [w for w in ws if isinstance(w, Q.QuantWeight)]

    def _partial(self, x: torch.Tensor, w, x16: torch.Tensor | None = None, x8=None):
        if isinstance(w, (torch.Tensor, gemm.PackedLinear)):
            fc = gemm.fused_choice(x.shape[0], w)
            return gemm.gemm_partial(x, w, fc) if fc is not None else None
        M = x.shape[0]
        if getattr(w, "v2", False) and x.is_cuda and (M <= Q.MAX_FUSED_M or (
                M <= Q.F8_DECODE_MAX_M and self.tp.world_size == 1 and Q.f8_decode_ok(w))):
            return Q.quant_partial(x, w, x16, x8)
        return None

    X16 = os.environ.get("HIPSERVE_QGEMM_X16", "1") != "0"

    def _x16(self, like: torch.Tensor, consumer):
        if (not self.X16 or self.tp.world_size != 1 or not like.is_cuda or not 32 < like.shape[0] <= 64
                or not getattr(consumer, "v2", False) or not hasattr(torch.ops.hipserve, "splitk_glu")
                or Q.f8_decode_ok(consumer)):
            return None
        return torch.empty(like.shape, dtype=torch.float16, device=like.device)

    def _x8p(self, like: torch.Tensor, consumer, glu: bool = False):
        if (self.tp.world_size != 1 or not like.is_cuda or isinstance(consumer, torch.Tensor)
                or getattr(self.ops, "name", "") != "hip" or not pgemm.f8_use(consumer, like.shape[0], glu)):
            return None
        return (torch.empty(like.shape, dtype=torch.uint8, device=like.device),
                torch.empty(like.shape[0], dtype=torch.float32, device=like.device))

    def _x8(self, like: torch.Tensor, consumer):
        if (self.tp.world_size != 1 or not like.is_cuda or like.shape[0] > Q.F8_DECODE_MAX_M
                or not Q.f8_decode_ok(consumer)):
            return None
        return (torch.empty(like.shape, dtype=torch.uint8, device=like.device),
                torch.empty(like.shape[0], dtype=torch.float32, device=like.device))

    def _decode_split(self, Td: int, meta: AttnMeta):
        part = self.decode_partition
        width = meta.bt_decode.shape[1] * self.block_size_hint
        if Td * self.nkv >= 512 or (Td * self.nkv >= 128 and width <= 2048):
            part = max(part, 2048)
        mp = max(1, -(-width // part))
        to, tm = meta.tmp_out, meta.tmp_ml
        if to is None or mp > to.shape[2]:
            return self.decode_partition, to, tm
        nq, D = to.shape[1], to.shape[3]
        to = to.view(-1)[: Td * nq * mp * D].view(Td, nq, mp, D)
        tm = tm.view(-1)[: Td * nq * mp * 2].view(Td, nq, mp, 2)
        return part, to, tm

    def compute_logits(self, hidden: torch.Tensor) -> torch.Tensor:
        logits = self.linear(hidden, self.lm_head)
        logits = self.tp.all_gather_lastdim(logits)
        return logits[:, : self.cfg.vocab_size]

    def kv_bytes_per_block(self, block_size: int) -> int:
        return 2 * self.cfg.num_layers * self.nkv * block_size * self.D * torch.finfo(self.kv_dtype).bits // 8

    def allocate_kv_cache(self, num_blocks: int, block_size: int):
        L = self.cfg.num_layers
        k = torch.zeros(L, num_blocks, self.nkv, block_size, self.D, device=self.device, dtype=self.kv_dtype)
        v = torch.zeros(L, num_blocks, self.nkv, self.D, block_size, device=self.device, dtype=self.kv_dtype)
        return [(k[i], v[i]) for i in range(L)]
```

hipserve/ops/__init__.py:

```python
from __future__ import annotations

import os
import threading

import torch

from . import reference as ref

_LIB = os.path.join(os.path.dirname(os.path.dirname(os.path.abspath(__file__))), "_C.so")
_lock = threading.Lock()
_loaded = False


def library_path() -> str:
    return _LIB


def load_library(build_if_missing: bool = False) -> str:
    global _loaded
    with _lock:
        if _loaded:
            return _LIB
        if not os.path.exists(_LIB) and build_if_missing:
            from .._build import build_kernels

            build_kernels()
        if not os.path.exists(_LIB):
            raise RuntimeError(
                f"hipserve native kernels not built ({_LIB} missing): run `python -m hipserve._build`")
        torch.ops.load_library(_LIB)
        _loaded = True
        return _LIB


def native_available() -> bool:
    try:
        load_library()
        return True
    except Exception:
        return False


class KernelOps:

    name = "hip"

    def __init__(self):
        load_library()
        self._op = torch.ops.hipserve

    def rmsnorm(self, out, x, w, eps, out8=None):
        self._op.rmsnorm(out, x, w, eps, *(out8 if out8 is not None else (None, None)))
        return out

    def fused_add_rmsnorm(self, out, x, residual, w, eps, out8=None):
        self._op.fused_add_rmsnorm(out, x, residual, w, eps, *(out8 if out8 is not None else (None, None)))
        return out

    def silu_and_mul(self, out, x):
        self._op.silu_and_mul(out, x)
        return out

    def gelu_and_mul(self, out, x):
        self._op.gelu_and_mul(out, x)
        return out

    def qk_rmsnorm(self, qkv, q_w, k_w, nq, nkv, D, eps):
        self._op.qk_rmsnorm(qkv, q_w, k_w, nq, nkv, D, eps)

    def fill_uniform(self, out, row0, col0, gcols, key, scale):
        self._op.fill_uniform(out, row0, col0, gcols, key, scale)
        return out

    def rope_cache(self, qkv, positions, slots, cos_sin, k_cache, v_cache, nq, nkv, D, mode):
        self._op.rope_cache(qkv, positions, slots, cos_sin, k_cache, v_cache, nq, nkv, D, mode)

    def paged_decode(self, out, q, k_cache, v_cache, block_tables, context_lens, tmp_out, tmp_ml,
                     nq, nkv, part_size, scale, window=0, out16=None):
        self._op.paged_decode(out, q, k_cache, v_cache, block_tables, context_lens, tmp_out, tmp_ml,
                              nq, nkv, part_size, scale, window, out16)
        return out

    def prefill_attention(self, out, q, k_cache, v_cache, block_tables, cu_q, ctx_lens, tiles,
                          nq, nkv, scale, window=0):
        self._op.prefill_attention(out, q, k_cache, v_cache, block_tables, cu_q, ctx_lens, tiles,
                                   nq, nkv, scale, window)
        return out

    def sample(self, out_tok, out_lp, logits, temperature, top_k, top_p, seeds, steps, two_rounds=True,
               min_p=None):
        self._op.sample(out_tok, out_lp, logits, temperature, top_k, top_p, seeds, steps, two_rounds, min_p)

    def penalty_apply(self, logits, slot, pres, freq, rep, counts, seen):
        self._op.penalty_apply(logits, slot, pres, freq, rep, counts, seen)

    def logit_bias_apply(self, logits, slot, ids, vals, n):
        self._op.logit_bias_apply(logits, slot, ids, vals, n)

    def penalty_update(self, tok, slot, counts, seen):
        self._op.penalty_update(tok, slot, counts, seen)

    def penalty_init(self, counts, seen, slots, off, n_prompt, toks):
        self._op.penalty_init(counts, seen, slots, off, n_prompt, toks)

    def top_logprobs(self, logits, nreq, out_ids, out_lp):
        self._op.top_logprobs(logits, nreq, out_ids, out_lp)

    def layernorm(self, out, x, w, b, eps, residual=None):
        self._op.layernorm(out, x, w, b, residual, eps)
        return out

    def gelu_(self, x, tanh):
        self._op.gelu_(x, tanh)
        return x

    VISION_TILE = 128

    def vision_meta(self, geo, nh, D):
        import numpy as np

        cu = geo.cu_seqlens
        tiles = np.array([(s, r) for s in range(len(cu) - 1) for r in range(0, int(cu[s + 1] - cu[s]),
                                                                          self.VISION_TILE)], np.int32)
        dev = torch.device("cuda", torch.cuda.current_device())
        return (torch.from_numpy(cu.astype(np.int32)).to(dev), torch.from_numpy(tiles.reshape(-1, 2)).to(dev))

    def vision_attention(self, out, qkv, cos_sin, cu_seqlens, nh, D, scale, meta=None):
        cu, tiles = meta
        self._op.vision_attention(out, qkv, cos_sin, cu, tiles, nh, D, scale)
        return out


class ReferenceOps:

    name = "reference"

    def fill_uniform(self, out, row0, col0, gcols, key, scale):
        return ref.fill_uniform(out, row0, col0, gcols, key, scale)

    def rmsnorm(self, out, x, w, eps, out8=None):
        assert out8 is None, "the FP8 copy is a HIP-kernel output"
        out.copy_(ref.rmsnorm(x, w, eps))
        return out

    def fused_add_rmsnorm(self, out, x, residual, w, eps, out8=None):
        assert out8 is None, "the FP8 copy is a HIP-kernel output"
        y, r = ref.fused_add_rmsnorm(x, residual, w, eps)
        residual.copy_(r)
        out.copy_(y)
        return out

    def silu_and_mul(self, out, x):
        out.copy_(ref.silu_and_mul(x))
        return out

    def gelu_and_mul(self, out, x):
        out.copy_(ref.gelu_and_mul(x))
        return out

    def qk_rmsnorm(self, qkv, q_w, k_w, nq, nkv, D, eps):
        ref.qk_rmsnorm(qkv, q_w, k_w, nq, nkv, D, eps)

    def rope_cache(self, qkv, positions, slots, cos_sin, k_cache, v_cache, nq, nkv, D, mode):
        ref.rope_cache(qkv, positions, slots, cos_sin, k_cache, v_cache, nq, nkv, D, mode)

    def paged_decode(self, out, q, k_cache, v_cache, block_tables, context_lens, tmp_out, tmp_ml,
                     nq, nkv, part_size, scale, window=0, out16=None):
        B = context_lens.shape[0]
        D = k_cache.shape[3]
        out[:B, : nq * D].copy_(ref.paged_decode(q, k_cache, v_cache, block_tables, context_lens,
                                                 nq, nkv, scale, window).view(B, nq * D))
        return out

    def prefill_attention(self, out, q, k_cache, v_cache, block_tables, cu_q, ctx_lens, tiles,
                          nq, nkv, scale, window=0):
        D = k_cache.shape[3]
        T = int(cu_q[-1])
        out[:T, : nq * D].copy_(ref.prefill_attention(q, k_cache, v_cache, block_tables, cu_q,
                                                      ctx_lens, nq, nkv, scale, window).view(T, nq * D))
        return out

    def penalty_apply(self, logits, slot, pres, freq, rep, counts, seen):
        ref.penalty_apply(logits, slot, pres, freq, rep, counts, seen)

    def logit_bias_apply(self, logits, slot, ids, vals, n):
        ref.logit_bias_apply(logits, slot, ids, vals, n)

    def penalty_update(self, tok, slot, counts, seen):
        ref.penalty_update(tok, slot, counts, seen)

    def penalty_init(self, counts, seen, slots, off, n_prompt, toks):
        ref.penalty_init(counts, seen, slots, off, n_prompt, toks)

    def top_logprobs(self, logits, nreq, out_ids, out_lp):
        ref.top_logprobs(logits, nreq, out_ids, out_lp)

    def layernorm(self, out, x, w, b, eps, residual=None):
        if residual is None:
            out.copy_(ref.layernorm(x, w, b, eps))
        else:
            y, r = ref.add_layernorm(x, residual, w, b, eps)
            residual.copy_(r)
            out.copy_(y)
        return out

    def gelu_(self, x, tanh):
        x.copy_(ref.gelu(x, tanh))
        return x

    def vision_attention(self, out, qkv, cos_sin, cu_seqlens, nh, D, scale, meta=None):
        ref.vision_rope(qkv, cos_sin, nh, D)
        out.copy_(ref.vision_attention(qkv, cu_seqlens, nh, D, scale))
        return out

    def sample(self, out_tok, out_lp, logits, temperature, top_k, top_p, seeds, steps, two_rounds=True,
               min_p=None):
        t, lp = ref.sample(logits, temperature, top_k, top_p, seeds, steps, bf16_row=False, min_p=min_p)
        n = t.shape[0]
        out_tok[:n].copy_(t)
        if out_lp.numel():
            out_lp[:n].copy_(lp)


def get_ops(device: torch.device | str):
    device = torch.device(device)
    if device.type == "cuda":
        return KernelOps()
    return ReferenceOps()
```

hipserve/ops/gemm.py:

```python
from __future__ import annotations

import logging
import weakref

import torch
import torch.nn.functional as F

log = logging.getLogger("hipserve.gemm")

SKINNY_CONFIGS = [(1, 1), (1, 2), (1, 4), (1, 8), (1, 16), (2, 1), (2, 2), (2, 4), (2, 8)]
SPLITK_CONFIGS = [1, 2, 4, 8]
DG_RT = [1, 2, 3]
DG_STEPS = [1, 2, 4, 7, 8, 12, 16, 21]
PACKED: dict[int, tuple] = {}
PACKED_GLU: dict[int, tuple] = {}
COLD_BYTES = 1 << 30
COLD_COPIES_MAX = 1024
TC_KIND = "decode_gemm_cold2"
_EMPTY = {}
TUNE_MS = [1, 2, 4, 8, 16, 24, 32, 48, 64]


class GemmTuner:
    def __init__(self):
# ... 135 lines not shown
                if K % (256 * ns):
                    continue
                sp = K // (256 * ns)
                if (sp > 1 and N % 8) or tiles * sp > 4096 or (tiles * sp < 64 and N * K > (1 << 21)):
                    continue
                out.append(("dg", rt, sp))
                if packed:
                    out.append(("dgp", rt, sp))
        for rt, kw in SKINNY_CONFIGS:
            if K % (256 * kw) == 0:
                out.append(("sk", rt, kw))
        return out


class _Unit:

    def __init__(self, spec, M, N, device):
        op = torch.ops.hipserve
        self.op, self.spec, self.M, self.N = op, spec, M, N
        bf = dict(device=device, dtype=torch.bfloat16)
        self.kind = spec[0]
        if self.kind == "norm":
            self.res = torch.randn(M, N, **bf)
            self.w = torch.ones(N, **bf)
            self.y = torch.empty(M, N, **bf)
        elif self.kind in ("rope", "attn"):
            _, self.nq, self.nkv, self.D, self.mode = spec
            nb = -(-M // 16) + 1
            self.kc = torch.zeros(nb, self.nkv, 16, self.D, **bf)
            self.vc = torch.zeros(nb, self.nkv, self.D, 16, **bf)
            self.pos = torch.arange(M, device=device, dtype=torch.long)
            self.slots = torch.arange(M, device=device, dtype=torch.long)
            self.cs = torch.rand(4096, self.D, device=device, dtype=torch.float32)
            self.qkv = torch.empty(M, N, **bf)
        elif self.kind == "glu":
            self.act = torch.empty(M, N // 2, **bf)

    def blas(self, y):
        op = self.op
        if self.kind == "norm":
            op.fused_add_rmsnorm(self.y, y, self.res, self.w, 1e-5)
        elif self.kind in ("rope", "attn"):
            op.rope_cache(y, self.pos, self.slots, self.cs, self.kc, self.vc, self.nq, self.nkv, self.D, self.mode)
        else:
            op.silu_and_mul(self.act, y)

    def fused(self, cfg, x, w, wp):
        op, M, N = self.op, self.M, self.N
        kind, rt, S = cfg
        packed = kind == "dgp" and wp is not None
        if self.kind == "glu":
            if packed:
                ws = torch.empty(S * M * N, dtype=torch.float32, device=x.device) if S > 1 else \
                    _empty(x.device)[1]
                op.decode_gemm_glu(self.act, x, wp, ws, N, rt, S)
            else:
                y = torch.empty(M, N, dtype=x.dtype, device=x.device)
                decode_gemm(y, x, w, rt, S)
                op.silu_and_mul(self.act, y)
            return
        ws = torch.empty(S * M * N, dtype=torch.float32, device=x.device)
        op.decode_gemm_partial(ws, x, wp if packed else w, N, rt, S, packed)
        if self.kind == "norm":
            op.splitk_add_rmsnorm(self.y, self.res, ws, S, self.w, 1e-5)
        elif self.kind == "attn":
            pass
        else:
            op.splitk_rope_cache(self.qkv, ws, S, self.pos, self.slots, self.cs, self.kc, self.vc,
                                 self.nq, self.nkv, self.D, self.mode)


TUNER = GemmTuner()


def _empty(device):
    e = _EMPTY.get(device)
    if e is None:
        e = _EMPTY[device] = (torch.empty(0, dtype=torch.int16, device=device),
                              torch.empty(0, dtype=torch.float32, device=device))
    return e


def splitk_gemm(out, x, w, splits):
    M, K = x.shape
    N = w.shape[0]
    e16, e32 = _empty(x.device)
    ws = torch.empty(splits, M, N, dtype=torch.float32, device=x.device) if splits > 1 else e32
    torch.ops.hipserve.gguf_gemm(out, x, w.view(torch.uint8), e16, e16, 6, 2 * K, N, K, ws, splits)
    return out


def decode_gemm(out, x, w, rt, splits):
    M, N = x.shape[0], w.shape[0]
    ws = (torch.empty(splits * M * N, dtype=torch.float32, device=x.device) if splits > 1
          else _empty(x.device)[1])
    torch.ops.hipserve.decode_gemm(out, x, w, ws, rt, splits)
    return out


def packable(N: int, K: int) -> bool:
    return K % 256 == 0 and N % 8 == 0


def pack(w: torch.Tensor, glu: bool = False) -> torch.Tensor:
    N, K = w.shape
    out = torch.empty(-(-N // 128) * 128 * K, dtype=w.dtype, device=w.device)
    torch.ops.hipserve.pack_decode_weight(out, w.contiguous(), glu)
    return out


class PackedLinear:

    def __init__(self, wp: torch.Tensor, N: int, K: int, glu: bool = False):
        self.wp, self.N, self.K, self.glu = wp, N, K, glu
        self.shape = (N, K)
        self.dtype, self.device = wp.dtype, wp.device
        self.is_cuda = wp.is_cuda

    def dim(self) -> int:
        return 2

    def numel(self) -> int:
        return self.N * self.K

    def element_size(self) -> int:
        return self.wp.element_size()

    def data_ptr(self) -> int:
        return self.wp.data_ptr()

    def unpack(self) -> torch.Tensor:
        T, KS = -(-self.N // 128), self.K // 256
        v = self.wp.view(T, KS, 8, 8, 4, 16, 8).permute(0, 2, 5, 1, 3, 4, 6).reshape(T, 128, self.K)
        if self.glu:
            v = v.view(T, 2, 64, self.K)
            return torch.cat([v[:, 0].reshape(-1, self.K), v[:, 1].reshape(-1, self.K)])[:self.N]
        return v.reshape(T * 128, self.K)[:self.N]

    def float(self) -> torch.Tensor:
        return self.unpack().float()

    def to(self, *a, **k) -> torch.Tensor:
        return self.unpack().to(*a, **k)

    def t(self) -> torch.Tensor:
        return self.unpack().t()


def _lookup(reg, w):
    e = reg.get(w.data_ptr())
    if e is None:
        return None
    ref, wp = e
    if ref() is not w:
        reg.pop(w.data_ptr(), None)
        return None
    return wp


def packed_of(w):
    if isinstance(w, PackedLinear):
        return None if w.glu else w.wp
    return _lookup(PACKED, w)


def glu_of(w):
    if isinstance(w, PackedLinear):
        return w.wp if w.glu else None
    return _lookup(PACKED_GLU, w)


def register_packed(w: torch.Tensor, glu: bool = False) -> torch.Tensor:
    reg = PACKED_GLU if glu else PACKED
    wp = _lookup(reg, w)
    if wp is None:
        wp = pack(w, glu)
        reg[w.data_ptr()] = (weakref.ref(w), wp)
    return wp


def decode_gemm_packed(out, x, wp, N, rt, splits):
    M = x.shape[0]
    ws = (torch.empty(splits * M * N, dtype=torch.float32, device=x.device) if splits > 1
          else _empty(x.device)[1])
    torch.ops.hipserve.decode_gemm_packed(out, x, wp, ws, N, rt, splits)
    return out


def fused_choice(M: int, w):
    if isinstance(w, PackedLinear):
        if M > 64 or w.glu:
            return None
        return TUNER.choose_packed(M, w.N, w.K), w.wp
    if not isinstance(w, torch.Tensor) or M > 64 or not TUNER.table:
        return None
    c = TUNER.choose(M, w.shape[0], w.shape[1])
    if not isinstance(c, tuple) or c[0] not in ("dg", "dgp"):
        return None
    wp = packed_of(w) if c[0] == "dgp" else None
    return c, wp


def gemm_partial(x, w, fc):
    (kind, rt, S), wp = fc
    M, N = x.shape[0], w.shape[0]
    ws = torch.empty(S * M * N, dtype=torch.float32, device=x.device)
    packed = wp is not None
    torch.ops.hipserve.decode_gemm_partial(ws, x, wp if packed else w, N, rt, S, packed)
    return ws, S


def glu_choice(M: int, w):
    if isinstance(w, PackedLinear):
        if M > 64 or not w.glu:
            return None
        c = TUNER.choose_packed(M, w.N, w.K)
        return c[1], c[2], w.wp
    if not isinstance(w, torch.Tensor) or M > 64 or not TUNER.table:
        return None
    c = TUNER.choose(M, w.shape[0], w.shape[1])
    wp = glu_of(w)
    if not isinstance(c, tuple) or c[0] != "dgp" or wp is None:
        return None
    return c[1], c[2], wp


def gemm_glu(x, w, gc):
    rt, S, wp = gc
    M, N = x.shape[0], w.shape[0]
    act = torch.empty(M, N // 2, dtype=x.dtype, device=x.device)
    ws = (torch.empty(S * M * N, dtype=torch.float32, device=x.device) if S > 1 else _empty(x.device)[1])
    torch.ops.hipserve.decode_gemm_glu(act, x, wp, ws, N, rt, S)
    return act


def run_choice(c, out, x, w, wp=None):
    if c[0] == "dgp":
        if wp is None:
            wp = packed_of(w)
        if wp is None:
            return decode_gemm(out, x, w, c[1], c[2])
        return decode_gemm_packed(out, x, wp, w.shape[0], c[1], c[2])
    if c[0] == "dg":
        return decode_gemm(out, x, w, c[1], c[2])
    if c[0] == "sk":
        torch.ops.hipserve.skinny_gemm(out, x, w, c[1], c[2])
        return out
    if c[0] == "splitk":
        return splitk_gemm(out, x, w, c[1])
    raise ValueError(c)


PW_WM = int(__import__("os").environ.get("HIPSERVE_PW_WM", "1"))
PW_RW = int(__import__("os").environ.get("HIPSERVE_PW_RW", "4"))
PW_GRID = int(__import__("os").environ.get("HIPSERVE_PW_GRID", str(1 << 30)))


def packed_prefill(x: torch.Tensor, w: PackedLinear, epi: int = 0, out: torch.Tensor | None = None,
                   bias: torch.Tensor | None = None) -> torch.Tensor:
    M = x.shape[0]
    if out is None:
        out = torch.empty(M, w.N // 2 if epi in (2, 3) else w.N, device=x.device, dtype=x.dtype)
    torch.ops.hipserve.prefill_gemm_packed(out, x, w.wp, w.N, epi, bias, PW_WM, PW_GRID, PW_RW)
    return out


def packed_linear(x: torch.Tensor, w: PackedLinear) -> torch.Tensor:
    assert not w.glu, "a GLU-interleaved weight has no plain x W^T (use packed_glu)"
    M = x.shape[0]
    if x.stride(1) != 1 or x.stride(0) % 8:
        x = x.contiguous()
    if M <= 64:
        c = TUNER.choose_packed(M, w.N, w.K)
        out = torch.empty(M, w.N, device=x.device, dtype=x.dtype)
        return decode_gemm_packed(out, x, w.wp, w.N, c[1], c[2])
    return packed_prefill(x, w)


def packed_glu(x: torch.Tensor, w: PackedLinear, gelu: bool = False) -> torch.Tensor:
    assert w.glu
    M = x.shape[0]
    if x.stride(1) != 1 or x.stride(0) % 8:
        x = x.contiguous()
    if M <= 64 and not gelu:
        c = TUNER.choose_packed(M, w.N, w.K)
        return gemm_glu(x, w, (c[1], c[2], w.wp))
    return packed_prefill(x, w, 3 if gelu else 2)


def linear(x: torch.Tensor, w: torch.Tensor) -> torch.Tensor:
    if isinstance(w, PackedLinear):
        return packed_linear(x, w)
    M = x.shape[0]
    if M <= 64 and x.is_cuda and TUNER.table:
        c = TUNER.choose(M, w.shape[0], w.shape[1])
        if c != "blas" and x.stride(1) == 1 and x.stride(0) % 8 == 0:
            out = torch.empty(M, w.shape[0], device=x.device, dtype=x.dtype)
            return run_choice(c, out, x, w)
    return F.linear(x, w)
```

hipserve/ops/reference.py:

```python
from __future__ import annotations

import math

import numpy as np
import torch


def rmsnorm(x: torch.Tensor, w: torch.Tensor, eps: float) -> torch.Tensor:
    xf = x.float()
    inv = torch.rsqrt(xf.pow(2).mean(-1, keepdim=True) + eps)
    return (xf * inv * w.float()).to(x.dtype)


def fused_add_rmsnorm(x: torch.Tensor, residual: torch.Tensor, w: torch.Tensor, eps: float):
    r = (x.float() + residual.float()).to(x.dtype)
    return rmsnorm(r, w, eps), r


def silu_and_mul(x: torch.Tensor) -> torch.Tensor:
    inter = x.shape[-1] // 2
    g, u = x[..., :inter].float(), x[..., inter:].float()
    return (torch.nn.functional.silu(g) * u).to(x.dtype)


def gelu_and_mul(x: torch.Tensor) -> torch.Tensor:
    inter = x.shape[-1] // 2
    g, u = x[..., :inter].float(), x[..., inter:].float()
    return (torch.nn.functional.gelu(g, approximate="tanh") * u).to(x.dtype)


def layernorm(x: torch.Tensor, w: torch.Tensor, b: torch.Tensor, eps: float) -> torch.Tensor:
    return torch.nn.functional.layer_norm(x.float(), (x.shape[-1],), w.float(), b.float(), eps).to(x.dtype)


def add_layernorm(x: torch.Tensor, residual: torch.Tensor, w, b, eps: float):
    r = (x.float() + residual.float()).to(x.dtype)
    return layernorm(r, w, b, eps), r


def gelu(x: torch.Tensor, tanh: bool) -> torch.Tensor:
    return torch.nn.functional.gelu(x.float(), approximate="tanh" if tanh else "none").to(x.dtype)


def vision_rope(qkv: torch.Tensor, cos_sin: torch.Tensor, nh: int, D: int):
    T = qkv.shape[0]
    half = D // 2
    c, s = cos_sin[:T, None, :half].float(), cos_sin[:T, None, half:].float()
    for j in range(2):
        x = qkv[:, j * nh * D:(j + 1) * nh * D].view(T, nh, D)
        a, b = x[..., :half].float(), x[..., half:].float()
        x.copy_(torch.cat([a * c - b * s, b * c + a * s], -1).to(x.dtype))


def vision_attention(qkv: torch.Tensor, cu_seqlens, nh: int, D: int, scale: float) -> torch.Tensor:
    T = qkv.shape[0]
    q = qkv[:, : nh * D].view(T, nh, D).float()
    k = qkv[:, nh * D:2 * nh * D].view(T, nh, D).float()
    v = qkv[:, 2 * nh * D:].view(T, nh, D).float()
    out = torch.empty(T, nh, D, dtype=torch.float32, device=qkv.device)
    cu = [int(x) for x in cu_seqlens]
    for a, b in zip(cu[:-1], cu[1:]):
        s = torch.einsum("qhd,khd->hqk", q[a:b], k[a:b]) * scale
        out[a:b] = torch.einsum("hqk,khd->qhd", torch.softmax(s, -1), v[a:b])
    return out.view(T, nh * D).to(qkv.dtype)


def qk_rmsnorm(qkv: torch.Tensor, q_w: torch.Tensor, k_w: torch.Tensor, nq: int, nkv: int, D: int, eps: float):
    T = qkv.shape[0]
    if T == 0:
        return
    q = qkv[:, : nq * D].view(T, nq, D)
    k = qkv[:, nq * D:(nq + nkv) * D].view(T, nkv, D)
    q.copy_(rmsnorm(q, q_w, eps))
    k.copy_(rmsnorm(k, k_w, eps))


def rope_cos_sin(head_dim: int, max_pos: int, theta: float, scaling: dict | None = None,
                 rotary_dim: int | None = None) -> torch.Tensor:
    rd = rotary_dim or head_dim
    inv_freq = 1.0 / (theta ** (torch.arange(0, rd, 2, dtype=torch.float64) / rd))
    if scaling and scaling.get("rope_type", scaling.get("type")) == "llama3":
        factor = scaling["factor"]
        lo, hi = scaling.get("low_freq_factor", 1.0), scaling.get("high_freq_factor", 4.0)
        old = scaling.get("original_max_position_embeddings", 8192)
        lo_wl, hi_wl = old / lo, old / hi
        wl = 2 * math.pi / inv_freq
        smooth = (old / wl - lo) / (hi - lo)
        scaled = torch.where(wl > lo_wl, inv_freq / factor, inv_freq)
        mid = (wl <= lo_wl) & (wl >= hi_wl)
        scaled = torch.where(mid, (1 - smooth) * inv_freq / factor + smooth * inv_freq, scaled)
        inv_freq = scaled
    elif scaling and scaling.get("rope_type", scaling.get("type")) == "linear":
        inv_freq = inv_freq / scaling["factor"]
    t = torch.arange(max_pos, dtype=torch.float64)
    f = torch.outer(t, inv_freq)
    return torch.cat([f.cos(), f.sin()], dim=-1).float().contiguous()


def apply_rope(x: torch.Tensor, pos: torch.Tensor, cos_sin: torch.Tensor, mode: int) -> torch.Tensor:
    D = x.shape[-1]
    half = D // 2
    cs = cos_sin[pos.long()]
    c, s = cs[:, None, :half], cs[:, None, half:]
    xf = x.float()
    if mode == 0:
        a, b = xf[..., :half], xf[..., half:]
        out = torch.cat([a * c - b * s, b * c + a * s], dim=-1)
    else:
        a, b = xf[..., 0::2], xf[..., 1::2]
        out = torch.stack([a * c - b * s, b * c + a * s], dim=-1).flatten(-2)
    return out.to(x.dtype)


def to_cache(x: torch.Tensor, dtype) -> torch.Tensor:
    if dtype == torch.float8_e4m3fn:
        return x.float().clamp(-448.0, 448.0).to(dtype)
    return x.to(dtype)


def rope_cache(qkv, positions, slots, cos_sin, k_cache, v_cache, nq, nkv, D, mode):
    T = qkv.shape[0]
    if T == 0:
        return
    q = qkv[:, : nq * D].view(T, nq, D)
    k = qkv[:, nq * D:(nq + nkv) * D].view(T, nkv, D)
    v = qkv[:, (nq + nkv) * D:(nq + 2 * nkv) * D].view(T, nkv, D)
    q.copy_(apply_rope(q, positions[:T], cos_sin, mode))
    kr = apply_rope(k, positions[:T], cos_sin, mode)
    bs = k_cache.shape[2]
    sl = slots[:T].long()
    valid = sl >= 0
    if valid.any():
        sv = sl[valid]
        blk, off = sv // bs, sv % bs
        k_cache[blk, :, off, :] = to_cache(kr[valid], k_cache.dtype)
        v_cache[blk, :, :, off] = to_cache(v[valid], v_cache.dtype)


def _gather_kv(k_cache, v_cache, block_table, n):
    bs = k_cache.shape[2]
    idx = torch.arange(n, device=k_cache.device)
    blk = block_table[(idx // bs)].long()
    off = idx % bs
    k = k_cache[blk, :, off, :]
    v = v_cache[blk, :, :, off]
    return k, v


def paged_decode(q, k_cache, v_cache, block_tables, context_lens, nq, nkv, scale, window=0):
    D = k_cache.shape[3]
    B = context_lens.shape[0]
    G = nq // nkv
    out = torch.empty(B, nq, D, dtype=q.dtype, device=q.device)
    for b in range(B):
        n = int(context_lens[b])
        k, v = _gather_kv(k_cache, v_cache, block_tables[b], n)
        if window > 0 and n > window:
            k, v = k[n - window:], v[n - window:]
        qb = q[b, : nq * D].view(nq, D).float()
        kf = k.float().repeat_interleave(G, dim=1)
        vf = v.float().repeat_interleave(G, dim=1)
        s = torch.einsum("hd,nhd->hn", qb, kf) * scale
        p = torch.softmax(s, dim=-1)
        out[b] = torch.einsum("hn,nhd->hd", p, vf).to(q.dtype)
    return out


def prefill_attention(q, k_cache, v_cache, block_tables, cu_q, ctx_lens, nq, nkv, scale, window=0):
    D = k_cache.shape[3]
    G = nq // nkv
    T = int(cu_q[-1])
    out = torch.empty(T, nq, D, dtype=q.dtype, device=q.device)
    for s_ in range(len(ctx_lens)):
        q0, q1 = int(cu_q[s_]), int(cu_q[s_ + 1])
        ql, ctx = q1 - q0, int(ctx_lens[s_])
        if ql == 0:
            continue
        k, v = _gather_kv(k_cache, v_cache, block_tables[s_], ctx)
        qs = q[q0:q1, : nq * D].view(ql, nq, D).float()
        kf = k.float().repeat_interleave(G, dim=1)
        vf = v.float().repeat_interleave(G, dim=1)
        s = torch.einsum("qhd,nhd->hqn", qs, kf) * scale
        qpos = torch.arange(ctx - ql, ctx, device=q.device)[:, None]
        kpos = torch.arange(ctx, device=q.device)[None, :]
        mask = kpos > qpos
        if window > 0:
            mask = mask | (kpos <= qpos - window)
        s = s.masked_fill(mask[None], float("-inf"))
        p = torch.softmax(s, dim=-1)
        out[q0:q1] = torch.einsum("hqn,nhd->qhd", p, vf).to(q.dtype)
    return out




def row_key(seed: int, step: int) -> int:
    M = (1 << 64) - 1
    x = ((seed & M) * 0x9E3779B97F4A7C15 & M) ^ (((step & M) + 0xD1B54A32D192ED03) & M) * 0xBF58476D1CE4E5B9 & M
    x ^= x >> 31
    x = x * 0x7FB5D329728EA185 & M
    x ^= x >> 27
    x = x * 0x81DADEF4BC2DD44D & M
    x ^= x >> 33
    return (x ^ (x >> 32)) & 0xFFFFFFFF


def uniform01(seed: int, step: int, n: int) -> np.ndarray:
    key = np.uint32(row_key(seed, step))
    with np.errstate(over="ignore"):
        i = np.arange(n, dtype=np.uint32)
        h = key ^ (i * np.uint32(0x9E3779B9) + np.uint32(0x7F4A7C15))
        h ^= h >> np.uint32(16)
        h *= np.uint32(0x85EBCA6B)
        h ^= h >> np.uint32(13)
        h *= np.uint32(0xC2B2AE35)
        h ^= h >> np.uint32(16)
    return (((h >> np.uint32(8)).astype(np.float64) + 0.5) / 16777216.0).astype(np.float32)


def sample_keep(x: torch.Tensor, t: float, k: int, p: float, mp: float = 0.0) -> torch.Tensor:
    V = x.shape[0]
    keep = torch.ones(V, dtype=torch.bool)
    if 0 < k < V:
        kth = torch.topk(x, k).values[-1]
        keep &= x >= kth
    if p < 1.0:
        w = torch.exp((x - x.max()) / t) * keep
        order = torch.argsort(x, descending=True)
        cum = torch.cumsum(w[order].double(), 0)
        target = p * float(cum[-1])
        n = int(torch.searchsorted(cum, torch.tensor([target], dtype=torch.float64))[0])
        thr = x[order[min(n, V - 1)]]
        keep &= x >= thr
    if mp > 0.0:
        keep &= (x - x.max()) / t >= min(math.log(mp), 0.0)
    return keep


def sample(logits: torch.Tensor, temperature, top_k, top_p, seeds, steps, bf16_row: bool = True, min_p=None):
    B, V = logits.shape
    toks = torch.empty(B, dtype=torch.long)
    lps = torch.empty(B, dtype=torch.float32)
    lf = logits.float().cpu()
    if bf16_row:
        lf = lf.to(torch.bfloat16).float()
    for r in range(B):
        x = lf[r]
        lse = torch.logsumexp(x, 0)
        t = float(temperature[r])
        if not t > 1e-5:
            i = int(torch.argmax(x))
            toks[r], lps[r] = i, float(x[i] - lse)
            continue
        keep = sample_keep(x, t, int(top_k[r]), float(top_p[r]), float(min_p[r]) if min_p is not None else 0.0)
        u = torch.from_numpy(uniform01(int(seeds[r]), int(steps[r]), V))
        g = (x - x.max()) / t - torch.log(-torch.log(u))
        g = torch.where(keep, g, torch.full_like(g, float("-inf")))
        i = int(torch.argmax(g))
        toks[r], lps[r] = i, float(x[i] - lse)
    return toks, lps


def _mix32(x: torch.Tensor) -> torch.Tensor:
    M = 0xFFFFFFFF
    x = x ^ (x >> 16)
    x = (x * 0x7FEB352D) & M
    x = x ^ (x >> 15)
    x = (x * 0x846CA68B) & M
    return x ^ (x >> 16)


def fill_uniform(out: torch.Tensor, row0: int, col0: int, gcols: int, key: int, scale: float):
    rows, cols = out.shape
    r = torch.arange(rows, dtype=torch.int64).unsqueeze(1) + row0
    c = torch.arange(cols, dtype=torch.int64).unsqueeze(0) + col0
    idx = (r * gcols + c) & 0xFFFFFFFF
    h = _mix32(_mix32(idx) ^ (key & 0xFFFFFFFF))
    u = (h >> 8).to(torch.float32) * 5.9604644775390625e-08
    v = (u - 0.5) * torch.tensor(2.0 * scale, dtype=torch.float32)
    out.copy_(v.to(torch.bfloat16).to(out.dtype))
# ... 86 lines not shown
```

Before: 7633.

## Compute last-layer attention and MLP only for logits rows during prefill

In the final transformer layer during prefill, K/V are still computed and written to the cache for every token, but Q projection, RoPE on Q, attention, and the MLP are applied only to the rows whose logits are needed. Attention for those rows runs through the paged decode kernel against the cache. The rope kernel gains a Q row range and a Q-only mode so unneeded Q rotation is skipped. This removes last-layer compute for prefill tokens whose hidden states are discarded, at the cost of extra index_select and a split QKV GEMM.

```diff
diff --git a/csrc/include/hipserve/kernels.h b/csrc/include/hipserve/kernels.h
--- a/csrc/include/hipserve/kernels.h
+++ b/csrc/include/hipserve/kernels.h
@@ -21,7 +21,8 @@
 void launch_rope_cache(void* qkv, long qkv_stride, const long* positions,
                        const long* slots, const float* cos_sin, void* k_cache,
                        void* v_cache, int T, int nq, int nkv, int D,
-                       int block_size, int mode, hipStream_t s, bool kv_f8 = false);
+                       int block_size, int mode, hipStream_t s, bool kv_f8 = false, int q_lo = 0,
+                       int q_hi = 1 << 30, bool write_kv = true);
 
 size_t paged_decode_smem_bytes(int D);
 void launch_paged_decode_qkv(void* out, long out_stride, const float* ws, int S, int N, const long* positions,
diff --git a/csrc/kernels/rope_cache.hip b/csrc/kernels/rope_cache.hip
--- a/csrc/kernels/rope_cache.hip
+++ b/csrc/kernels/rope_cache.hip
@@ -22,10 +22,13 @@
     const long* __restrict__ positions, const long* __restrict__ slots,
     const float* __restrict__ cos_sin, KV* __restrict__ k_cache,
     KV* __restrict__ v_cache, int nq, int nkv, int D,
-    int block_size) {
+    int block_size, int q_lo, int q_hi, int write_kv) {
   const int t = blockIdx.x;
+  const long slot = write_kv ? slots[t] : -1;
+  const int h_lo = t >= q_lo && t < q_hi ? 0 : nq;
+  const int h_hi = slot >= 0 ? nq + nkv : nq;
+  if (h_hi <= h_lo) return;
   const long pos = positions[t];
-  const long slot = slots[t];
   const int half = D / 2;
   const float* cs = cos_sin + pos * D;
   unsigned short* row = qkv + t * qkv_stride;
@@ -34,9 +37,9 @@
 
   if constexpr (kMode == 0) {
     const int chunks = half / 8;
-    const int items = (nq + nkv) * chunks;
+    const int items = (h_hi - h_lo) * chunks;
     for (int it = threadIdx.x; it < items; it += blockDim.x) {
-      const int h = it / chunks, c = it % chunks;
+      const int h = h_lo + it / chunks, c = it % chunks;
       unsigned short* base = row + h * D;
       u16x8 va = *reinterpret_cast<u16x8*>(base + c * 8);
       u16x8 vb = *reinterpret_cast<u16x8*>(base + half + c * 8);
@@ -49,7 +52,7 @@
       if (h < nq) {
         *reinterpret_cast<u16x8*>(base + c * 8) = va;
         *reinterpret_cast<u16x8*>(base + half + c * 8) = vb;
-      } else if (slot >= 0) {
+      } else {
         const int kh = h - nq;
         KV* kc = k_cache + ((blk * nkv + kh) * block_size + off) * (long)D;
         kv_store8(kc + c * 8, va);
@@ -58,9 +61,9 @@
     }
   } else {
     const int chunks = D / 8;
-    const int items = (nq + nkv) * chunks;
+    const int items = (h_hi - h_lo) * chunks;
     for (int it = threadIdx.x; it < items; it += blockDim.x) {
-      const int h = it / chunks, c = it % chunks;
+      const int h = h_lo + it / chunks, c = it % chunks;
       unsigned short* base = row + h * D;
       u16x8 v = *reinterpret_cast<u16x8*>(base + c * 8);
 #pragma unroll
@@ -75,7 +78,7 @@
       }
       if (h < nq) {
         *reinterpret_cast<u16x8*>(base + c * 8) = v;
-      } else if (slot >= 0) {
+      } else {
         const int kh = h - nq;
         KV* kc = k_cache + ((blk * nkv + kh) * block_size + off) * (long)D;
         kv_store8(kc + c * 8, v);
@@ -101,7 +104,8 @@
 __global__ __launch_bounds__(256) void rope_cache_tile_kernel(
     unsigned short* __restrict__ qkv, long qkv_stride, const long* __restrict__ positions,
     const long* __restrict__ slots, const float* __restrict__ cos_sin, KV* __restrict__ k_cache,
-    KV* __restrict__ v_cache, int T, int nq, int nkv, int D, int block_size, int vfast) {
+    KV* __restrict__ v_cache, int T, int nq, int nkv, int D, int block_size, int vfast, int q_lo, int q_hi,
+    int write_kv) {
   extern __shared__ __attribute__((aligned(16))) unsigned short vs[];
   const int t0 = blockIdx.x * kRopeTile;
   const int nt = min(kRopeTile, T - t0);
@@ -112,8 +116,11 @@
   for (int it = threadIdx.x; it < nt * per_tok; it += blockDim.x) {
     const int tt = it / per_tok, c = (it % per_tok) >> 1, hpar = it & 1;
     const int t = t0 + tt;
+    const long slot = write_kv ? slots[t] : -1;
+    const int h_lo = t >= q_lo && t < q_hi ? 0 : nq;
+    const int h_hi = slot >= 0 ? nh : nq;
+    if (h_hi <= h_lo) continue;
     const long pos = positions[t];
-    const long slot = slots[t];
     const float* cs = cos_sin + pos * D;
     unsigned short* row = qkv + t * qkv_stride;
     const long blk = slot >= 0 ? slot / block_size : 0;
@@ -122,18 +129,18 @@
       float co[8], si[8];
 #pragma unroll
       for (int j = 0; j < 8; ++j) { co[j] = cs[c * 8 + j]; si[j] = cs[half + c * 8 + j]; }
-      for (int h0 = hpar; h0 < nh; h0 += 8) {
+      for (int h0 = h_lo + hpar; h0 < h_hi; h0 += 8) {
         u16x8 va[4], vb[4];
 #pragma unroll
         for (int q = 0; q < 4; ++q) {
-          const int h = min(h0 + 2 * q, nh - 1);
+          const int h = min(h0 + 2 * q, h_hi - 1);
           va[q] = *reinterpret_cast<const u16x8*>(row + h * D + c * 8);
           vb[q] = *reinterpret_cast<const u16x8*>(row + h * D + half + c * 8);
         }
 #pragma unroll
         for (int q = 0; q < 4; ++q) {
           const int h = h0 + 2 * q;
-          if (h >= nh || (h >= nq && slot < 0)) continue;
+          if (h >= h_hi) continue;
 #pragma unroll
           for (int j = 0; j < 8; ++j) {
             float ra, rb;
@@ -155,15 +162,15 @@
       float co[4], si[4];
 #pragma unroll
       for (int p = 0; p < 4; ++p) { co[p] = cs[c * 4 + p]; si[p] = cs[half + c * 4 + p]; }
-      for (int h0 = hpar; h0 < nh; h0 += 8) {
+      for (int h0 = h_lo + hpar; h0 < h_hi; h0 += 8) {
         u16x8 v[4];
 #pragma unroll
         for (int q = 0; q < 4; ++q)
-          v[q] = *reinterpret_cast<const u16x8*>(row + min(h0 + 2 * q, nh - 1) * D + c * 8);
+          v[q] = *reinterpret_cast<const u16x8*>(row + min(h0 + 2 * q, h_hi - 1) * D + c * 8);
 #pragma unroll
         for (int q = 0; q < 4; ++q) {
           const int h = h0 + 2 * q;
-          if (h >= nh || (h >= nq && slot < 0)) continue;
+          if (h >= h_hi) continue;
 #pragma unroll
           for (int p = 0; p < 4; ++p) {
             float ra, rb;
@@ -177,6 +184,7 @@
       }
     }
   }
+  if (!write_kv) return;
   const int VW = nkv * D, VR = VW + 8;
   const int vchunks = VW / 8;
   for (int it = threadIdx.x; it < nt * vchunks; it += blockDim.x) {
@@ -231,38 +239,41 @@
 template <typename KV>
 static void rope_cache_t(unsigned short* q, long qkv_stride, const long* positions, const long* slots,
                          const float* cos_sin, KV* kc, KV* vc, int T, int nq, int nkv, int D, int block_size,
-                         int mode, hipStream_t s) {
+                         int mode, hipStream_t s, int q_lo, int q_hi, int write_kv) {
   if (T >= 2048 && nkv * D <= 2048 && rope_tile_enabled()) {
     const dim3 tg((T + kRopeTile - 1) / kRopeTile);
     const size_t smem = (size_t)kRopeTile * (nkv * D + 8) * sizeof(unsigned short);
     if (mode == 0)
       rope_cache_tile_kernel<0, KV><<<tg, 256, smem, s>>>(q, qkv_stride, positions, slots, cos_sin, kc, vc, T, nq,
-                                                          nkv, D, block_size, rope_vfast());
+                                                          nkv, D, block_size, rope_vfast(), q_lo, q_hi, write_kv);
     else
       rope_cache_tile_kernel<1, KV><<<tg, 256, smem, s>>>(q, qkv_stride, positions, slots, cos_sin, kc, vc, T, nq,
-                                                          nkv, D, block_size, rope_vfast());
+                                                          nkv, D, block_size, rope_vfast(), q_lo, q_hi, write_kv);
     return;
   }
   if (mode == 0)
     rope_cache_kernel<0, KV><<<T, 256, 0, s>>>(q, qkv_stride, positions, slots, cos_sin, kc, vc, nq, nkv, D,
-                                               block_size);
+                                               block_size, q_lo, q_hi, write_kv);
   else
     rope_cache_kernel<1, KV><<<T, 256, 0, s>>>(q, qkv_stride, positions, slots, cos_sin, kc, vc, nq, nkv, D,
-                                               block_size);
+                                               block_size, q_lo, q_hi, write_kv);
 }
 
 void launch_rope_cache(void* qkv, long qkv_stride, const long* positions,
                        const long* slots, const float* cos_sin, void* k_cache,
                        void* v_cache, int T, int nq, int nkv, int D,
-                       int block_size, int mode, hipStream_t s, bool kv_f8) {
-  if (T <= 0) return;
+                       int block_size, int mode, hipStream_t s, bool kv_f8, int q_lo, int q_hi,
+                       bool write_kv) {
+  q_lo = q_lo < 0 ? 0 : q_lo;
+  q_hi = nq <= 0 ? q_lo : q_hi > T ? T : q_hi;
+  if (T <= 0 || (!write_kv && q_hi <= q_lo)) return;
   auto* q = static_cast<unsigned short*>(qkv);
   if (kv_f8)
     rope_cache_t(q, qkv_stride, positions, slots, cos_sin, static_cast<unsigned char*>(k_cache),
-                 static_cast<unsigned char*>(v_cache), T, nq, nkv, D, block_size, mode, s);
+                 static_cast<unsigned char*>(v_cache), T, nq, nkv, D, block_size, mode, s, q_lo, q_hi, write_kv);
   else
     rope_cache_t(q, qkv_stride, positions, slots, cos_sin, static_cast<unsigned short*>(k_cache),
-                 static_cast<unsigned short*>(v_cache), T, nq, nkv, D, block_size, mode, s);
-}
-
-}
+                 static_cast<unsigned short*>(v_cache), T, nq, nkv, D, block_size, mode, s, q_lo, q_hi, write_kv);
+}
+
+}
diff --git a/csrc/torch_bindings.cpp b/csrc/torch_bindings.cpp
--- a/csrc/torch_bindings.cpp
+++ b/csrc/torch_bindings.cpp
@@ -397,15 +397,31 @@
 
 void rope_cache(at::Tensor& qkv, const at::Tensor& positions, const at::Tensor& slots,
                 const at::Tensor& cos_sin, at::Tensor& k_cache, at::Tensor& v_cache,
-                int64_t nq, int64_t nkv, int64_t head_dim, int64_t mode) {
+                int64_t nq, int64_t nkv, int64_t head_dim, int64_t mode, int64_t q_lo, int64_t q_hi) {
   Args a("rope_cache", qkv, "qkv");
   TORCH_CHECK(head_dim > 0 && head_dim % 16 == 0 && (mode == 0 || mode == 1), "rope_cache: head_dim % 16 == 0, mode 0 / 1");
+  TORCH_CHECK(nq >= 0 && nkv > 0, "rope_cache: nq >= 0, nkv > 0");
   void* qp = a.ptr(qkv, "qkv", BF16, ROWS, {ANY, at_least((nq + 2 * nkv) * head_dim)});
   const int T = qkv.size(0);
+  if (q_hi < 0) q_hi = T;
+  TORCH_CHECK(0 <= q_lo && q_hi <= T, "rope_cache: the q row range must lie in [0, ", T, "]");
   const RopeArgs r = rope_args(a, positions, slots, cos_sin, T, head_dim);
   const KvCache kv = kv_cache(a, k_cache, v_cache, nkv, head_dim);
   hipserve::launch_rope_cache(qp, qkv.stride(0), r.positions, r.slots, r.cos_sin, kv.k, kv.v, T, nq, nkv, head_dim,
-                              kv.bs, mode, cur_stream(), kv.f8);
+                              kv.bs, mode, cur_stream(), kv.f8, (int)q_lo, (int)q_hi, true);
+}
+
+void rope_q(at::Tensor& q, const at::Tensor& positions, const at::Tensor& cos_sin, int64_t nq, int64_t head_dim,
+            int64_t mode) {
+  Args a("rope_q", q, "q");
+  TORCH_CHECK(head_dim > 0 && head_dim % 16 == 0 && (mode == 0 || mode == 1), "rope_q: head_dim % 16 == 0, mode 0 / 1");
+  TORCH_CHECK(nq > 0, "rope_q: nq > 0");
+  void* qp = a.ptr(q, "q", BF16, ROWS, {ANY, at_least(nq * head_dim)});
+  const int T = q.size(0);
+  const int64_t* pp = a.as<int64_t>(positions, "positions", CONTIG, T);
+  const float* cs = a.as<float>(cos_sin, "cos_sin", CONTIG, {ANY, head_dim});
+  hipserve::launch_rope_cache(qp, q.stride(0), pp, nullptr, cs, nullptr, nullptr, T, nq, 0, head_dim, 16, mode,
+                              cur_stream(), false, 0, T, false);
 }
 
 void paged_decode(at::Tensor& out, const at::Tensor& q, const at::Tensor& k_cache,
@@ -1228,7 +1244,8 @@
                    "Tensor weight, float eps, float scale=1.0, Tensor(c!)? out8=None, Tensor(d!)? xs8=None) -> ()") \
   X(fused_add_rmsnorm, "(Tensor(a!) out, Tensor x, Tensor(b!) residual, Tensor weight, float eps, Tensor(c!)? out8=None, Tensor(d!)? xs8=None) -> ()") \
   X(silu_and_mul, "(Tensor(a!) out, Tensor x) -> ()") \
-  X(rope_cache, "(Tensor(a!) qkv, Tensor positions, Tensor slots, Tensor cos_sin, Tensor(b!) k_cache, Tensor(c!) v_cache, int nq, int nkv, int head_dim, int mode) -> ()") \
+  X(rope_cache, "(Tensor(a!) qkv, Tensor positions, Tensor slots, Tensor cos_sin, Tensor(b!) k_cache, Tensor(c!) v_cache, int nq, int nkv, int head_dim, int mode, int q_lo=0, int q_hi=-1) -> ()") \
+  X(rope_q, "(Tensor(a!) q, Tensor positions, Tensor cos_sin, int nq, int head_dim, int mode) -> ()") \
   X(paged_decode, "(Tensor(a!) out, Tensor q, Tensor k_cache, Tensor v_cache, Tensor block_tables, Tensor context_lens, Tensor(b!) tmp_out, Tensor(c!) tmp_ml, int nq, int nkv, int part_size, float scale, int window=0, Tensor(d!)? out16=None) -> ()") \
   X(prefill_attention, "(Tensor(a!) out, Tensor q, Tensor k_cache, Tensor v_cache, Tensor block_tables, Tensor cu_q, Tensor ctx_lens, Tensor tiles, int nq, int nkv, float scale, int window=0) -> ()") \
   X(qk_rmsnorm, "(Tensor(a!) qkv, Tensor q_w, Tensor k_w, int nq, int nkv, int head_dim, float eps) -> ()") \
diff --git a/hipserve/engine/model_runner.py b/hipserve/engine/model_runner.py
--- a/hipserve/engine/model_runner.py
+++ b/hipserve/engine/model_runner.py
@@ -119,6 +119,7 @@
                     tp.calibrate_collectives(H, ecfg.max_num_batched_tokens)
         self.init_times["collectives_s"] = round(time.time() - t1, 2)
         self.max_bs = min(ecfg.max_num_seqs, max(GRAPH_BUCKETS))
+        self.prefill_tail = bool(ecfg.extra.get("prefill_tail", True))
         self.buckets = [b for b in GRAPH_BUCKETS if b <= max(self.max_bs, 1)]
         if self.buckets[-1] < self.max_bs:
             self.buckets.append(self.max_bs)
@@ -562,11 +563,14 @@
             meta.tmp_ml = torch.empty(inp.num_decode, *self.tmp_ml.shape[1:], device=self.device)
         if "mm" in inp.extra:
             self._attach_mm(inp.extra["mm"], meta, len(inp.ids))
+        rows = self._t(inp.logits_rows)
+        if self.prefill_tail and inp.num_prefill_tokens:
+            self._attach_tail(inp, meta, rows)
+        tail = hasattr(self.model, "prefill_tail_ok") and self.model.prefill_tail_ok(meta)
         hidden = self.model.forward(ids, meta, self.kv)
         if n == 0:
             return np.zeros(0, np.int64), np.zeros(0, np.float32), None
-        rows = self._t(inp.logits_rows)
-        logits = self.model.compute_logits(hidden.index_select(0, rows))
+        logits = self.model.compute_logits(hidden if tail else hidden.index_select(0, rows))
         top = None
         if inp.top_logprobs:
             ti = torch.empty(n, TOP_LOGPROBS, dtype=torch.int32, device=self.device)
@@ -592,6 +596,17 @@
         if inp.top_logprobs:
             top = (ti.cpu().numpy(), tl.cpu().numpy())
         return tok.cpu().numpy(), lp.cpu().numpy(), top
+
+    def _attach_tail(self, inp: StepInputs, meta: AttnMeta, rows: torch.Tensor):
+        n_pf = len(inp.logits_rows) - inp.num_decode
+        seq = np.searchsorted(inp.cu_q, inp.logits_rows[:n_pf], side="right") - 1
+        bt, ctx = inp.bt_prefill[seq], inp.ctx_prefill[seq]
+        if inp.num_decode:
+            bt, ctx = np.concatenate([bt, inp.bt_decode]), np.concatenate([ctx, inp.ctx_decode])
+        meta.tail_rows, meta.tail_bt, meta.tail_ctx = rows, self._t(bt), self._t(ctx.astype(np.int32))
+        if len(inp.logits_rows) > self.max_bs and meta.tmp_out is self.tmp_out:
+            meta.tmp_out = torch.empty(len(inp.logits_rows), *self.tmp_out.shape[1:], device=self.device)
+            meta.tmp_ml = torch.empty(len(inp.logits_rows), *self.tmp_ml.shape[1:], device=self.device)
 
     def _attach_mm(self, mm: dict, meta: AttnMeta, T: int):
         from ..models.vision import image_geometry
diff --git a/hipserve/models/llama.py b/hipserve/models/llama.py
--- a/hipserve/models/llama.py
+++ b/hipserve/models/llama.py
@@ -34,6 +34,9 @@
     mm_embeds: torch.Tensor | None = None
     mm_deepstack: list | None = None
     id_src: tuple | None = None
+    tail_rows: torch.Tensor | None = None
+    tail_bt: torch.Tensor | None = None
+    tail_ctx: torch.Tensor | None = None
 
 
 @dataclass
@@ -564,54 +567,100 @@
         x8 = self._x8p(xn, self.layers[0].wqkv)
         ops.rmsnorm(xn, h, self.layers[0].ln1, eps, out8=x8)
         L = len(self.layers)
+        tail = self.prefill_tail_ok(meta)
         for i, lw in enumerate(self.layers):
-            if x8 is not None:
-                qkv = pgemm.f8_gemm(xn, lw.wqkv, 0, x8=x8)
-            else:
-                qkv = self.linear(xn, lw.wqkv)
-            if lw.bqkv is not None:
-                qkv += lw.bqkv
-            if lw.q_norm is not None:
-                ops.qk_rmsnorm(qkv, lw.q_norm, lw.k_norm, nq, nkv, D, eps)
             kc, vc = kv_caches[i]
             win = cfg.window_of(i)
-            ops.rope_cache(qkv, meta.positions, meta.slot_mapping, self.cos_sin_local if win else cos_sin,
-                           kc, vc, nq, nkv, D, cfg.rope_mode)
+            cs = self.cos_sin_local if win else cos_sin
+            if tail and i == L - 1:
+                return self._prefill_tail(lw, xn, residual, x8, meta, kc, vc, cs, win)
+            qkv = self._qkv(xn, lw, x8)
+            ops.rope_cache(qkv, meta.positions, meta.slot_mapping, cs, kc, vc, nq, nkv, D, cfg.rope_mode)
             if Tp:
                 ops.prefill_attention(attn[:Tp], qkv[:Tp], kc, vc, meta.bt_prefill, meta.cu_q,
                                       meta.ctx_prefill, meta.tiles, nq, nkv, self.scale, win)
             if Td:
                 ops.paged_decode(attn[Tp:Tp + Td], qkv[Tp:Tp + Td], kc, vc, meta.bt_decode, meta.ctx_decode,
                                  tmp_out, tmp_ml, nq, nkv, part, self.scale, win)
-            x8 = self._x8p(xn, lw.wgu, glu=True)
-            self._rowpar_norm(xn, residual, attn, lw.wo, lw.post_attn_norm, lw.ln2, x8)
-            nxt = self.layers[i + 1].ln1 if i + 1 < L else self.norm
-            x8n = self._x8p(xn, self.layers[i + 1].wqkv) if i + 1 < L else None
-            act = h = None
-            if lw.router is not None:
-                h = self.moe(xn, lw)
-            else:
-                gelu = cfg.hidden_act == "gelu_tanh"
-                if pgemm.f8_use(lw.wgu, T, glu=True):
-                    act8 = None
-                    if pgemm.f8_use(lw.wd, T):
-                        act8 = pgemm.f8_glu_q8(xn, lw.wgu, gelu, x8)
-                    if act8 is not None:
-                        h = pgemm.f8_gemm(None, lw.wd, 0, x8=act8)
-                    else:
-                        act = pgemm.f8_gemm(xn, lw.wgu, 3 if gelu else 2, x8=x8)
-                elif isinstance(lw.wgu, gemm.PackedLinear) and lw.wgu.glu:
-                    act = gemm.packed_glu(xn, lw.wgu, gelu)
-                elif cfg.hidden_act in ("silu", "gelu_tanh") and Q.qprefill_ok(lw.wgu, T, glu=True):
-                    act = Q.qprefill(xn, lw.wgu, 3 if gelu else 2)
-                if act is None and h is None:
-                    gu = self.linear(xn, lw.wgu)
-                    act = torch.empty(T, self.inter, device=xn.device, dtype=xn.dtype)
-                    self.act_and_mul(act, gu)
             add = (meta.mm_rows, ds[i]) if ds is not None and i < len(ds) else None
-            self._rowpar_norm(xn, residual, act, lw.wd, lw.post_ff_norm, nxt, x8n, h, add)
-            x8 = x8n
+            x8 = self._post_attention(i, lw, xn, residual, attn, add)
         return xn
+
+    def _qkv(self, xn, lw: LayerWeights, x8):
+        if x8 is not None:
+            qkv = pgemm.f8_gemm(xn, lw.wqkv, 0, x8=x8)
+        else:
+            qkv = self.linear(xn, lw.wqkv)
+        if lw.bqkv is not None:
+            qkv += lw.bqkv
+        if lw.q_norm is not None:
+            self.ops.qk_rmsnorm(qkv, lw.q_norm, lw.k_norm, self.nq, self.nkv, self.D, self.cfg.rms_norm_eps)
+        return qkv
+
+    def _post_attention(self, i: int, lw: LayerWeights, xn, residual, attn, add=None):
+        cfg, L, T = self.cfg, len(self.layers), xn.shape[0]
+        x8 = self._x8p(xn, lw.wgu, glu=True)
+        self._rowpar_norm(xn, residual, attn, lw.wo, lw.post_attn_norm, lw.ln2, x8)
+        nxt = self.layers[i + 1].ln1 if i + 1 < L else self.norm
+        x8n = self._x8p(xn, self.layers[i + 1].wqkv) if i + 1 < L else None
+        act = h = None
+        if lw.router is not None:
+            h = self.moe(xn, lw)
+        else:
+            gelu = cfg.hidden_act == "gelu_tanh"
+            if pgemm.f8_use(lw.wgu, T, glu=True):
+                act8 = None
+                if pgemm.f8_use(lw.wd, T):
+                    act8 = pgemm.f8_glu_q8(xn, lw.wgu, gelu, x8)
+                if act8 is not None:
+                    h = pgemm.f8_gemm(None, lw.wd, 0, x8=act8)
+                else:
+                    act = pgemm.f8_gemm(xn, lw.wgu, 3 if gelu else 2, x8=x8)
+            elif isinstance(lw.wgu, gemm.PackedLinear) and lw.wgu.glu:
+                act = gemm.packed_glu(xn, lw.wgu, gelu)
+            elif cfg.hidden_act in ("silu", "gelu_tanh") and Q.qprefill_ok(lw.wgu, T, glu=True):
+                act = Q.qprefill(xn, lw.wgu, 3 if gelu else 2)
+            if act is None and h is None:
+                gu = self.linear(xn, lw.wgu)
+                act = torch.empty(T, self.inter, device=xn.device, dtype=xn.dtype)
+                self.act_and_mul(act, gu)
+        self._rowpar_norm(xn, residual, act, lw.wd, lw.post_ff_norm, nxt, x8n, h, add)
+        return x8n
+
+    def prefill_tail_ok(self, meta: AttnMeta) -> bool:
+        ds = meta.mm_deepstack if meta.mm_rows is not None else None
+        return (meta.tail_rows is not None and meta.num_prefill_tokens > 0 and bool(self.layers)
+                and not (ds is not None and len(self.layers) - 1 < len(ds)))
+
+    def _prefill_tail(self, lw: LayerWeights, xn, residual, x8, meta: AttnMeta, kc, vc, cs, win):
+        ops, cfg = self.ops, self.cfg
+        D, nq, nkv = self.D, self.nq, self.nkv
+        rows, L = meta.tail_rows, len(self.layers)
+        split = isinstance(lw.wqkv, torch.Tensor) and x8 is None and lw.q_norm is None
+        if split:
+            kv = self.linear(xn, lw.wqkv[nq * D:])
+            if lw.bqkv is not None:
+                kv += lw.bqkv[nq * D:]
+            ops.rope_cache(kv, meta.positions, meta.slot_mapping, cs, kc, vc, 0, nkv, D, cfg.rope_mode)
+        else:
+            qkv = self._qkv(xn, lw, x8)
+            ops.rope_cache(qkv, meta.positions, meta.slot_mapping, cs, kc, vc, nq, nkv, D, cfg.rope_mode, 0, 0)
+        R = rows.shape[0]
+        if R == 0:
+            return xn[:0]
+        xr, rr = xn.index_select(0, rows), residual.index_select(0, rows)
+        if split:
+            q = self.linear(xr, lw.wqkv[:nq * D])
+            if lw.bqkv is not None:
+                q += lw.bqkv[:nq * D]
+        else:
+            q = qkv.index_select(0, rows)[:, :nq * D]
+        ops.rope_q(q, meta.positions.index_select(0, rows), cs, nq, D, cfg.rope_mode)
+        attn = torch.empty(R, nq * D, device=xn.device, dtype=xn.dtype)
+        part, tmp_out, tmp_ml = self._decode_split(R, meta, meta.tail_bt)
+        ops.paged_decode(attn, q, kc, vc, meta.tail_bt, meta.tail_ctx, tmp_out, tmp_ml, nq, nkv, part, self.scale, win)
+        self._post_attention(L - 1, lw, xr, rr, attn)
+        return xr
 
     def act_and_mul(self, out: torch.Tensor, gu: torch.Tensor):
         if self.cfg.hidden_act == "gelu_tanh":
@@ -750,9 +799,9 @@
         return (torch.empty(like.shape, dtype=torch.uint8, device=like.device),
                 torch.empty(like.shape[0], dtype=torch.float32, device=like.device))
 
-    def _decode_split(self, Td: int, meta: AttnMeta):
+    def _decode_split(self, Td: int, meta: AttnMeta, bt: torch.Tensor | None = None):
         part = self.decode_partition
-        width = meta.bt_decode.shape[1] * self.block_size_hint
+        width = (meta.bt_decode if bt is None else bt).shape[1] * self.block_size_hint
         if Td * self.nkv >= 512 or (Td * self.nkv >= 128 and width <= 2048):
             part = max(part, 2048)
         mp = max(1, -(-width // part))
diff --git a/hipserve/ops/__init__.py b/hipserve/ops/__init__.py
--- a/hipserve/ops/__init__.py
+++ b/hipserve/ops/__init__.py
@@ -72,8 +72,11 @@
         self._op.fill_uniform(out, row0, col0, gcols, key, scale)
         return out
 
-    def rope_cache(self, qkv, positions, slots, cos_sin, k_cache, v_cache, nq, nkv, D, mode):
-        self._op.rope_cache(qkv, positions, slots, cos_sin, k_cache, v_cache, nq, nkv, D, mode)
+    def rope_cache(self, qkv, positions, slots, cos_sin, k_cache, v_cache, nq, nkv, D, mode, q_lo=0, q_hi=-1):
+        self._op.rope_cache(qkv, positions, slots, cos_sin, k_cache, v_cache, nq, nkv, D, mode, q_lo, q_hi)
+
+    def rope_q(self, q, positions, cos_sin, nq, D, mode):
+        self._op.rope_q(q, positions, cos_sin, nq, D, mode)
 
     def paged_decode(self, out, q, k_cache, v_cache, block_tables, context_lens, tmp_out, tmp_ml,
                      nq, nkv, part_size, scale, window=0, out16=None):
@@ -161,8 +164,11 @@
     def qk_rmsnorm(self, qkv, q_w, k_w, nq, nkv, D, eps):
         ref.qk_rmsnorm(qkv, q_w, k_w, nq, nkv, D, eps)
 
-    def rope_cache(self, qkv, positions, slots, cos_sin, k_cache, v_cache, nq, nkv, D, mode):
-        ref.rope_cache(qkv, positions, slots, cos_sin, k_cache, v_cache, nq, nkv, D, mode)
+    def rope_cache(self, qkv, positions, slots, cos_sin, k_cache, v_cache, nq, nkv, D, mode, q_lo=0, q_hi=-1):
+        ref.rope_cache(qkv, positions, slots, cos_sin, k_cache, v_cache, nq, nkv, D, mode, q_lo, q_hi)
+
+    def rope_q(self, q, positions, cos_sin, nq, D, mode):
+        ref.rope_q(q, positions, cos_sin, nq, D, mode)
 
     def paged_decode(self, out, q, k_cache, v_cache, block_tables, context_lens, tmp_out, tmp_ml,
                      nq, nkv, part_size, scale, window=0, out16=None):
diff --git a/hipserve/ops/gemm.py b/hipserve/ops/gemm.py
--- a/hipserve/ops/gemm.py
+++ b/hipserve/ops/gemm.py
@@ -311,10 +311,10 @@
     if e is None:
         return None
     ref, wp = e
-    if ref() is not w:
+    if ref() is None:
         reg.pop(w.data_ptr(), None)
         return None
-    return wp
+    return wp if ref() is w else None
 
 
 def packed_of(w):
diff --git a/hipserve/ops/reference.py b/hipserve/ops/reference.py
--- a/hipserve/ops/reference.py
+++ b/hipserve/ops/reference.py
@@ -118,14 +118,22 @@
     return x.to(dtype)
 
 
-def rope_cache(qkv, positions, slots, cos_sin, k_cache, v_cache, nq, nkv, D, mode):
+def rope_q(q, positions, cos_sin, nq, D, mode):
+    T = q.shape[0]
+    if T:
+        qv = q[:, : nq * D].view(T, nq, D)
+        qv.copy_(apply_rope(qv, positions[:T], cos_sin, mode))
+
+
+def rope_cache(qkv, positions, slots, cos_sin, k_cache, v_cache, nq, nkv, D, mode, q_lo=0, q_hi=-1):
     T = qkv.shape[0]
     if T == 0:
         return
-    q = qkv[:, : nq * D].view(T, nq, D)
     k = qkv[:, nq * D:(nq + nkv) * D].view(T, nkv, D)
     v = qkv[:, (nq + nkv) * D:(nq + 2 * nkv) * D].view(T, nkv, D)
-    q.copy_(apply_rope(q, positions[:T], cos_sin, mode))
+    q_hi = T if q_hi < 0 else q_hi
+    if nq and q_hi > q_lo:
+        rope_q(qkv[q_lo:q_hi], positions[q_lo:q_hi], cos_sin, nq, D, mode)
     kr = apply_rope(k, positions[:T], cos_sin, mode)
     bs = k_cache.shape[2]
     sl = slots[:T].long()
```

New measurement: 7690 (median of 3 runs). No clear change (+0.7%).
